# gafniguy/4D-Facial-Avatars

Hardware: AMD Instinct MI355X
Metric: rays/sec at 512x512, 64 coarse + 128 fine samples (higher is better)
Workload: dtype f32; 1 GPU; configs[1]: paper-model eval forward, 512x512 frame, 64+128 samples, chunksize 65536, perturb on, expression+latent conditioned, background prior; frames sharded over GPUs

## Files before the change

### 4d-facial-avatars_amd/build.py

```python
from __future__ import annotations

import os
import shutil
import subprocess
import sys

HERE = os.path.dirname(os.path.abspath(__file__))
SRC = os.path.join(HERE, "csrc")
OUT_DIR = os.path.join(HERE, "lib")
OUT = os.path.join(OUT_DIR, "libnerface_hip.so")
SOURCES = ["nf_lib.hip", "nf_rays.hip", "nf_choice.hip", "nf_render.hip", "nf_render_bwd_full.hip", "nf_mlp.hip", "nf_mlp_bwd.hip", "nf_mlp_bf16.hip", "nf_mlp_f16.hip", "nf_mlp_f16x2.hip", "nf_mlp_f16_train.hip", "nf_mlp_f16_bwd.hip", "nf_mlp_f16_dw.hip", "nf_mlp_bf16_train.hip", "nf_mlp_bf16_bwd.hip", "nf_mlp_bf16_dw.hip", "nf_tiny.hip", "nf_flex.hip", "nf_mlp_lcode.hip", "nf_mlp_lcode_bwd.hip", "nf_mlp_lcode_bf16.hip", "nf_mlp_lcode_f16.hip", "nf_mlp_lcode_f16x2.hip", "nf_mlp_lcode_f16_train.hip", "nf_mlp_lcode_f16_bwd.hip", "nf_mlp_lcode_bf16_train.hip", "nf_mlp_lcode_bf16_bwd.hip", "nf_mlp_bshape.hip", "nf_mlp_cbshape.hip", "nf_mlp_smaller.hip", "nf_mlp_smaller_bwd.hip", "nf_pipeline.hip", "nf_mlp_encoded.hip", "nf_optim.hip", "nf_metrics.hip",
           "nf_mlp_sigma.hip", "nf_mlp_sigma_bf16.hip", "nf_mlp_sigma_f16.hip", "nf_mlp_sigma_f16x2.hip", "nf_mlp_lcode_sigma.hip",
           "nf_mlp_lcode_sigma_bf16.hip", "nf_mlp_lcode_sigma_f16.hip", "nf_mlp_lcode_sigma_f16x2.hip", "nf_mlp_smaller_sigma.hip",
           "nf_mlp_live.hip",
           "nf_mlp_live_stats.hip",
           "nf_mlp_gated.hip", "nf_mlp_gated_stats.hip",
           "nf_isosurface.hip",
           "nf_sparse_grid.hip",
           "nf_mesh_components.hip"]
FLAGS = ["--offload-arch=gfx950", "-O3", "-std=c++17", "-ffp-contract=off", "-fPIC", "-fvisibility=default",
         "-Wno-unused-result"]


UNIT_FLAGS = {u: ["-fno-slp-vectorize"] for u in ("nf_mlp_f16.hip", "nf_mlp_f16x2.hip", "nf_mlp_f16_train.hip", "nf_mlp_lcode_f16.hip",
                                                  "nf_mlp_lcode_f16x2.hip", "nf_mlp_lcode_f16_train.hip", "nf_mlp_sigma_f16.hip",
                                                  "nf_mlp_sigma_f16x2.hip", "nf_mlp_lcode_sigma_f16.hip", "nf_mlp_lcode_sigma_f16x2.hip")}
UNIT_FLAGS.update({u: ["-mllvm", "-amdgpu-atomic-optimizer-strategy=None"] for u in ("nf_mlp_live.hip", "nf_mlp_live_stats.hip",
                                                                                            "nf_mlp_gated.hip", "nf_mlp_gated_stats.hip")})


def _hipcc() -> str:
    for cand in (os.environ.get("HIPCC"), shutil.which("hipcc"), "/opt/rocm/bin/hipcc"):
        if cand and os.path.exists(cand):
            return cand
    raise RuntimeError("hipcc not found (need ROCm's hipcc to build libnerface_hip.so)")


def _stale() -> bool:
    if not os.path.exists(OUT):
        return True
    t = os.path.getmtime(OUT)
    deps = [os.path.join(SRC, f) for f in os.listdir(SRC)] + [os.path.join(HERE, "..", "include", "nerface_hip.h"), __file__]
    return any(os.path.getmtime(d) > t for d in deps)


def _includes(src: str, seen=None) -> set:
    import re
    seen = set() if seen is None else seen
    if src in seen or not os.path.exists(src):
        return seen
    seen.add(src)
    for m in re.finditer(r'^\s*#\s*include\s+"([^"]+)"', open(src).read(), re.M):
        _includes(os.path.normpath(os.path.join(os.path.dirname(src), m.group(1))), seen)
    return seen


def build(force: bool = False, verbose: bool = True) -> str:
    if not force and not _stale():
        return OUT
    os.makedirs(OUT_DIR, exist_ok=True)
    obj_dir = os.path.join(OUT_DIR, "obj")
    os.makedirs(obj_dir, exist_ok=True)
    objs = []
    cc = _hipcc()
    procs = []
    for s in SOURCES:
        src = os.path.join(SRC, s)
        if not os.path.exists(src):
            continue
        obj = os.path.join(obj_dir, s.replace(".hip", ".o"))
        objs.append(obj)
        newest = max(os.path.getmtime(d) for d in _includes(src) | {os.path.abspath(__file__)})
        if not force and os.path.exists(obj) and os.path.getmtime(obj) > newest:
            continue
        procs.append((s, subprocess.Popen([cc, *FLAGS, *UNIT_FLAGS.get(s, []), "-Rpass-analysis=kernel-resource-usage", "-c", src, "-o", obj],
                                          stdout=subprocess.PIPE, stderr=subprocess.STDOUT)))
    for s, p in procs:
        try:
            out, _ = p.communicate(timeout=900)
        except subprocess.TimeoutExpired:
            p.kill()
            raise RuntimeError(f"hipcc timed out on {s}")
        if p.returncode != 0:
            raise RuntimeError(f"hipcc failed on {s}:\n{out.decode()}")
        text = out.decode()
        usage = [ln for ln in text.splitlines() if "-Rpass-analysis=kernel-resource-usage" in ln]
        with open(os.path.join(obj_dir, s.replace(".hip", ".usage.txt")), "w") as f:
            f.write("\n".join(usage) + "\n")
        rest = "\n".join(ln for ln in text.splitlines() if "kernel-resource-usage" not in ln and not ln.lstrip().startswith(("|", "^", "In file included from"))
                         and not ln.strip()[:1].isdigit())
        if verbose and rest.strip():
            print(rest)
    cmd = [cc, "--offload-arch=gfx950", "-shared", "-fPIC", *objs, "-o", OUT]
    r = subprocess.run(cmd, stdout=subprocess.PIPE, stderr=subprocess.STDOUT)
    if r.returncode != 0:
        raise RuntimeError("link failed:\n" + r.stdout.decode())
    if verbose:
        print("built", OUT)
    return OUT


def build_tools(verbose: bool = True):
    micro = os.path.normpath(os.path.join(HERE, "..", "tools", "micro"))
    built = []
    for name in ("store_bw",):
        src, exe = os.path.join(micro, name + ".hip"), os.path.join(micro, name)
        if os.path.exists(exe) and os.path.getmtime(exe) > os.path.getmtime(src):
            continue
        r = subprocess.run([_hipcc(), "--offload-arch=gfx950", "-O2", "-Wno-unused-result", "-o", exe, src], stdout=subprocess.PIPE, stderr=subprocess.STDOUT)
        if r.returncode != 0:
            raise RuntimeError(f"hipcc failed on {src}:\n" + r.stdout.decode())
        built.append(exe)
        if verbose:
            print("built", exe)
    return built


if __name__ == "__main__":
    build(force="--force" in sys.argv)
    build_tools()
```

### 4d-facial-avatars_amd/csrc/nf_mlp_live_kernel.h

```cpp
#pragma once
#include <mutex>
#include "nf_mlp_paper_net.h"

#define NF_LIVE_ROWS 64
#ifndef NF_LIVE_PF
#define NF_LIVE_PF 8
#endif
#define NF_LIVE_DIR_B (NF_LIVE_ROWS * 1024)
#define NF_LIVE_META_B (NF_LIVE_DIR_B + NF_LIVE_ROWS * 64)
#define NF_LIVE_WAVE_B (NF_LIVE_META_B + NF_LIVE_ROWS * 16)
#define NF_LIVE_OOB NF_LIVE_WAVE_B
#define NF_LIVE_SC1 16

static_assert(NF_LIVE_ROWS == 64 && NF_MLP_NT == 2, "row numbers wrap with & 63; a pass's liveness is one 32-bit mask");
static_assert(NF_LIVE_PF >= 0 && NF_LIVE_PF <= 16, "prefetched rows live in registers beside fc_alpha's weights");

__device__ __forceinline__ __amdgpu_buffer_rsrc_t nf_live_ring(char* ring_v) {
    const uint64_t a = (uint64_t)ring_v;
    const uint64_t s = (uint64_t)(uint32_t)__builtin_amdgcn_readfirstlane((int)(uint32_t)a) |
                       ((uint64_t)(uint32_t)__builtin_amdgcn_readfirstlane((int)(a >> 32)) << 32);
    return __builtin_amdgcn_make_buffer_rsrc(reinterpret_cast<char*>(s), (short)0, NF_LIVE_WAVE_B, 0x00020000);
}
__device__ __forceinline__ void nf_live_store(__amdgpu_buffer_rsrc_t ring, int off_b, f32x4 v) {
    __builtin_amdgcn_raw_buffer_store_b128(__builtin_bit_cast(nf_u32x4, v), ring, off_b, 0, 0);
}
__device__ __forceinline__ f32x4 nf_live_load(__amdgpu_buffer_rsrc_t ring, int off_b) {
    return __builtin_bit_cast(f32x4, __builtin_amdgcn_raw_buffer_load_b128(ring, off_b, 0, NF_LIVE_SC1));
}
__device__ __forceinline__ int nf_live_pop(unsigned& m) {
    const int r = __builtin_ctz(m);
    m &= m - 1u;
    return r;
}
__device__ __forceinline__ int nf_live_slab(int prow, int lane) { return nf_act_idx4(prow, lane); }

struct NfLivePre {
    NfStream<NF_MLP_NT>& st;
    f32x4 (&wd)[16];
    f32x4 (&pf)[NF_LIVE_PF > 0 ? NF_LIVE_PF : 1];
    char* ring_v;
    int head_v, tail_v;
    __device__ __forceinline__ void wait() const {
        __builtin_amdgcn_fence(__ATOMIC_RELEASE, "workgroup");
        __builtin_amdgcn_s_waitcnt(0x0F70);
        __builtin_amdgcn_fence(__ATOMIC_ACQUIRE, "workgroup");
    }
    __device__ __forceinline__ void loads(const NfW& Wi, const NfW& Ci, int lane) {
        using Net = NfPaperNet;
        const __amdgpu_buffer_rsrc_t ring = nf_live_ring(ring_v);
        const int tail = __builtin_amdgcn_readfirstlane(tail_v), cnt = __builtin_amdgcn_readfirstlane(head_v) - tail;
#pragma unroll
        for (int i = 0; i < NF_LIVE_PF; ++i)
            pf[i] = nf_live_load(ring, i < cnt ? ((tail + i) & (NF_LIVE_ROWS - 1)) * 1024 + lane * 16 : NF_LIVE_OOB);
        nf_load_bias<8>(st.bias, Ci, Net::B_D0, lane);
        nf_load_w16<8>(st.wa, Wi, Net::OFF_D0 / 4, lane);
        nf_load_w16<8>(wd, Wi, Net::OFF_D0 / 4 + 16 * 9 * 64, lane);
        __builtin_amdgcn_sched_barrier(0);
    }
};

struct NfGatePre {
    NfStream<NF_MLP_NT>& st;
    f32x4 (&pf)[NF_LIVE_PF > 0 ? NF_LIVE_PF : 1];
    char* ring_v;
    int head_v, tail_v;
    const float* bound_v;
    __device__ __forceinline__ NfW image() const {
        const uint64_t a = (uint64_t)bound_v;
        const uint64_t s = (uint64_t)(uint32_t)__builtin_amdgcn_readfirstlane((int)(uint32_t)a) |
                           ((uint64_t)(uint32_t)__builtin_amdgcn_readfirstlane((int)(a >> 32)) << 32);
        return nf_w_image(reinterpret_cast<const float*>(s), NF_BOUND_FLOATS);
    }
    __device__ __forceinline__ void wait() const {
        __builtin_amdgcn_fence(__ATOMIC_RELEASE, "workgroup");
        __builtin_amdgcn_s_waitcnt(0x0F70);
        __builtin_amdgcn_fence(__ATOMIC_ACQUIRE, "workgroup");
    }
    __device__ __forceinline__ void loads(const NfW& Wi, const NfW& Ci, int lane) {
        using Net = NfPaperNet;
        const __amdgpu_buffer_rsrc_t ring = nf_live_ring(ring_v);
        const int tail = __builtin_amdgcn_readfirstlane(tail_v), cnt = __builtin_amdgcn_readfirstlane(head_v) - tail;
#pragma unroll
        for (int i = 0; i < NF_LIVE_PF; ++i)
            pf[i] = nf_live_load(ring, i < cnt ? ((tail + i) & (NF_LIVE_ROWS - 1)) * 1024 + lane * 16 : NF_LIVE_OOB);
        nf_load_bias<16>(st.bias, Ci, Net::B_FEAT, lane);
        nf_load_w16<16>(st.wa, Wi, Net::OFF_FEAT / 4, lane);
        __builtin_amdgcn_sched_barrier(0);
    }
};

#define NF_LIVE_STAT_UNITS 0
#define NF_LIVE_STAT_RUNS 1
#define NF_LIVE_STAT_FLUSH 2
#define NF_LIVE_STAT_CLOCK 3
#define NF_GATE_STAT_PROVEN 4
#define NF_LIVE_PH_TRUNK 0
#define NF_LIVE_PH_TILE 1
#define NF_LIVE_PH_APPEND 2
#define NF_LIVE_PH_ENTRY 3
#define NF_LIVE_PH_RUN 4
#define NF_LIVE_PH_DEAD 5
#define NF_LIVE_PHASES 6
#define NF_LIVE_STAT_COLS 4
#define NF_GATE_STAT_COLS 5

template <bool STATS, int COLS = NF_LIVE_STAT_COLS>
__device__ __forceinline__ void nf_live_stat(long long* stats, int col, long long add, bool set = false) {
    if constexpr (STATS) {
        const int cols = COLS + (((uintptr_t)stats & 1) ? NF_LIVE_PHASES : 0);
        stats = reinterpret_cast<long long*>((uintptr_t)stats & ~(uintptr_t)7);
        if ((threadIdx.x & 63) == 0) {
            long long* at = stats + ((size_t)blockIdx.x * NF_MLP_WAVES + (threadIdx.x >> 6)) * cols + col;
            if (set) *at = add;
            else (void)__hip_atomic_fetch_add(at, add, __ATOMIC_RELAXED, __HIP_MEMORY_SCOPE_AGENT);
        }
    }
}

template <bool STATS, int COLS>
__device__ __forceinline__ void nf_live_mark(long long* stats, int end, int start) {
    if constexpr (STATS) {
        if ((uintptr_t)stats & 1) {
            __builtin_amdgcn_sched_barrier(0);
            const long long t = (long long)__builtin_amdgcn_s_memtime();
            if ((threadIdx.x & 63) == 0) {
                long long* row = reinterpret_cast<long long*>((uintptr_t)stats & ~(uintptr_t)7) +
                                 ((size_t)blockIdx.x * NF_MLP_WAVES + (threadIdx.x >> 6)) * (COLS + NF_LIVE_PHASES) + COLS;
                if (end >= 0) (void)__hip_atomic_fetch_add(row + end, t, __ATOMIC_RELAXED, __HIP_MEMORY_SCOPE_AGENT);
                if (start >= 0) (void)__hip_atomic_fetch_add(row + start, -t, __ATOMIC_RELAXED, __HIP_MEMORY_SCOPE_AGENT);
            }
            __builtin_amdgcn_sched_barrier(0);
        }
    }
}
template <class Pre, int COLS>
struct NfMarkedPre : Pre {
    long long* stats;
    __device__ __forceinline__ void wait() const {
        nf_live_mark<true, COLS>(stats, NF_LIVE_PH_TRUNK, NF_LIVE_PH_TILE);
        Pre::wait();
    }
};

template <int NT, bool STATS, bool GATE = false>
__global__ void __launch_bounds__(64 * NF_MLP_WAVES, 1)
k_paper_mlp_fwd_live(const float* __restrict__ packed, const float* __restrict__ cond_, const float* __restrict__ ro,
                     const float* __restrict__ rd, const float* __restrict__ rd_view, const float* __restrict__ z,
                     int64_t n_points, int S, float* __restrict__ raw, float* __restrict__ scratch, unsigned* __restrict__ counter,
                     long long* __restrict__ stats, const float* __restrict__ bound) {
    using Net = NfPaperNet;
    constexpr int COLS = GATE ? NF_GATE_STAT_COLS : NF_LIVE_STAT_COLS;
    __shared__ __attribute__((aligned(16))) f32x4 lds[NF_MLP_WAVES * 16 * NT * 64];
    const int lane = threadIdx.x & 63, wave = threadIdx.x >> 6;
    f32x4* act4 = lds + wave * (16 * NT * 64);
    typedef __attribute__((address_space(1))) f32x4 nf_gf32x4;
    nf_gf32x4* raw_v = (nf_gf32x4*)raw;
    asm volatile("" : "+v"(raw_v));
    char* ring_v = reinterpret_cast<char*>(scratch) + ((size_t)blockIdx.x * NF_MLP_WAVES + wave) * NF_LIVE_WAVE_B;
    asm volatile("" : "+v"(ring_v));
    const float* z_v = z;
    const float* rdv_v = rd_view;
    asm volatile("" : "+v"(z_v), "+v"(rdv_v));
    const float* bound_v = bound;
    if constexpr (GATE) asm volatile("" : "+v"(bound_v));
    int head_v = 0, tail_v = 0;
    asm volatile("" : "+v"(head_v), "+v"(tail_v));
    typedef __attribute__((address_space(1))) unsigned nf_gu32;
    nf_gu32* ctr_v = (nf_gu32*)counter;
    asm volatile("" : "+v"(ctr_v));
    unsigned unit_v = 0;
    if (lane == 0) unit_v = __hip_atomic_fetch_add(ctr_v, 1u, __ATOMIC_RELAXED, __HIP_MEMORY_SCOPE_AGENT);
    asm volatile("" : "+v"(unit_v));
#pragma unroll 1
    for (;;) {
        const int64_t p0 = (int64_t)(uint32_t)__builtin_amdgcn_readfirstlane((int)unit_v) * (16 * NT);
        int64_t p0_v = p0;
        asm volatile("" : "+v"(p0_v));
        int more_v = p0 < n_points;
        asm volatile("" : "+v"(more_v));
        const bool more = __builtin_amdgcn_readfirstlane(more_v) != 0;
        unsigned next_v = 0;
        if (more && lane == 0) next_v = __hip_atomic_fetch_add(ctr_v, 1u, __ATOMIC_RELAXED, __HIP_MEMORY_SCOPE_AGENT);
        if (more) nf_live_stat<STATS, COLS>(stats, NF_LIVE_STAT_UNITS, 1);
        int opaque0 = 0;
        asm volatile("" : "+s"(opaque0));
        const NfW Wi = nf_w_image(packed + opaque0, Net::PACKED), Ci = nf_w_image(cond_ + opaque0, Net::COND_FLOATS);
        NfStream<NT> st;
        f32x4 wd[16], pf[NF_LIVE_PF > 0 ? NF_LIVE_PF : 1];
        f32x4 dirf[NT][1];
        float sigma_own[NT];
        float tag_own[NT] = {};
        bool proven[NT] = {};
        int live_v = 0, run_v = 0;
        if (more) {
            nf_live_mark<STATS, COLS>(stats, -1, NF_LIVE_PH_TRUNK);
            f32x4 pe[NT][4];
            nf_net_inputs<NT>(pe, dirf, p0, n_points, S, lane, ro, rd, rdv_v, z_v);
            f32x4 acc[NT][16];
            if constexpr (GATE) {
                if constexpr (STATS)
                    nf_paper_net_body<Net, NT, 1, true, NfMarkedPre<NfGatePre, COLS>, true>(
                        acc, sigma_own, pe, dirf, Wi, Ci, act4, lane, NfMarkedPre<NfGatePre, COLS>{{st, pf, ring_v, head_v, tail_v, bound_v}, stats});
                else
                    nf_paper_net_body<Net, NT, 1, true, NfGatePre, true>(acc, sigma_own, pe, dirf, Wi, Ci, act4, lane,
                                                                         NfGatePre{st, pf, ring_v, head_v, tail_v, bound_v});
#pragma unroll
                for (int t = 0; t < NT; ++t) {
                    const float s = acc[t][8].x, u = acc[t][8].y;
                    sigma_own[t] = nf_add(s, nf_mul(u, 0x1p-13f));
                    proven[t] = sigma_own[t] < -0x1p-100f && s > -INFINITY && u < INFINITY;
                }
            } else if constexpr (STATS) {
                nf_paper_net_body<Net, NT, 1, true>(acc, sigma_own, pe, dirf, Wi, Ci, act4, lane,
                                                    NfMarkedPre<NfLivePre, COLS>{{st, wd, pf, ring_v, head_v, tail_v}, stats});
            } else {
                nf_paper_net_body<Net, NT, 1, true>(acc, sigma_own, pe, dirf, Wi, Ci, act4, lane, NfLivePre{st, wd, pf, ring_v, head_v, tail_v});
            }
            nf_live_mark<STATS, COLS>(stats, NF_LIVE_PH_TILE, NF_LIVE_PH_APPEND);
            int lane_o = lane;
            asm volatile("" : "+v"(lane_o));
            const int g = lane_o >> 4, c = lane_o & 15;
            unsigned live = 0;
            int S_o = S;
            asm volatile("" : "+v"(S_o));
            const int64_t p0_o = (int64_t)(uint32_t)__builtin_amdgcn_readfirstlane((int)(uint32_t)p0_v) |
                                 ((int64_t)__builtin_amdgcn_readfirstlane((int)(p0_v >> 32)) << 32);
#pragma unroll
            for (int t = 0; t < NT; ++t) {
                const int64_t p = p0_o + 16 * t + c;
                bool is_live;
                if constexpr (GATE) {
                    const bool last = (p + 1) % S_o == 0;
                    is_live = g == 0 && p < n_points && (!proven[t] || last);
                    tag_own[t] = __int_as_float(last ? 1 : 0);
                } else {
                    is_live = g == 0 && p < n_points && (!(sigma_own[t] <= 0.0f) || (p + 1) % S_o == 0);
                }
                live |= ((unsigned)__builtin_amdgcn_ballot_w64(is_live) & 0xffffu) << (16 * t);
            }
            const int head = __builtin_amdgcn_readfirstlane(head_v), cnt = head - __builtin_amdgcn_readfirstlane(tail_v);
            const int n_live = __builtin_popcount(live);
            live_v = (int)live;
            if constexpr (GATE) {
                const int64_t left = n_points - p0_o;
                nf_live_stat<STATS, COLS>(stats, NF_GATE_STAT_PROVEN, (left < 16 * NT ? (int)left : 16 * NT) - n_live);
            }
            if (cnt + n_live >= 16 * NT) {
                run_v = 1;
            } else {
                const __amdgpu_buffer_rsrc_t ring = nf_live_ring(ring_v);
                unsigned mm = live;
#pragma unroll 1
                for (int i = 0; i < n_live; i += 4) {
                    f32x4 v[4];
                    int off[4];
#pragma unroll
                    for (int u = 0; u < 4; ++u) {
                        const bool ok = i + u < n_live;
                        const int r = ok ? nf_live_pop(mm) : 0;
                        off[u] = ok ? ((head + i + u) & (NF_LIVE_ROWS - 1)) * 1024 + lane_o * 16 : NF_LIVE_OOB;
                        v[u] = act4[nf_live_slab(r, lane_o)];
                    }
#pragma unroll
                    for (int u = 0; u < 4; ++u) nf_live_store(ring, off[u], v[u]);
                }
#pragma unroll
                for (int t = 0; t < NT; ++t) {
                    const int bit = 16 * t + c;
                    if ((live >> bit) & 1u) {
                        const int row = (head + __builtin_popcount(live & ((1u << bit) - 1u))) & (NF_LIVE_ROWS - 1);
                        nf_live_store(ring, NF_LIVE_DIR_B + row * 64 + g * 16, dirf[t][0]);
                        if (g == 0) {
                            const int64_t p = p0_o + bit;
                            nf_live_store(ring, NF_LIVE_META_B + row * 16,
                                          (f32x4){__int_as_float((int)(uint32_t)p), __int_as_float((int)(p >> 32)), GATE ? tag_own[t] : sigma_own[t], 0.0f});
                        }
                    }
                }
                head_v = head + n_live;
                asm volatile("" : "+v"(head_v));
            }
            nf_live_mark<STATS, COLS>(stats, NF_LIVE_PH_APPEND, -1);
        } else {
            if constexpr (GATE) {
                NfGatePre pre{st, pf, ring_v, head_v, tail_v, bound_v};
                pre.wait();
                pre.loads(Wi, Ci, lane);
            } else {
                NfLivePre pre{st, wd, pf, ring_v, head_v, tail_v};
                pre.wait();
                pre.loads(Wi, Ci, lane);
            }
#pragma unroll
            for (int t = 0; t < NT; ++t) {
                dirf[t][0] = (f32x4){0.0f, 0.0f, 0.0f, 0.0f};
                sigma_own[t] = 0.0f;
            }
            run_v = __builtin_amdgcn_readfirstlane(head_v) != __builtin_amdgcn_readfirstlane(tail_v) ? 2 : 0;
        }
        asm volatile("" : "+v"(live_v), "+v"(run_v));
        const int run = __builtin_amdgcn_readfirstlane(run_v);
        if (run != 0) {
            nf_live_stat<STATS, COLS>(stats, NF_LIVE_STAT_RUNS, 1);
            if (run == 2) nf_live_stat<STATS, COLS>(stats, NF_LIVE_STAT_FLUSH, __builtin_amdgcn_readfirstlane(head_v) - __builtin_amdgcn_readfirstlane(tail_v));
            nf_live_mark<STATS, COLS>(stats, -1, NF_LIVE_PH_ENTRY);
            int lane_o = lane;
            asm volatile("" : "+v"(lane_o));
            const int g = lane_o >> 4, c = lane_o & 15;
            const __amdgpu_buffer_rsrc_t ring = nf_live_ring(ring_v);
            const int tail = __builtin_amdgcn_readfirstlane(tail_v), cnt = __builtin_amdgcn_readfirstlane(head_v) - tail;
            const unsigned own = run == 1 ? (unsigned)__builtin_amdgcn_readfirstlane(live_v) : 0u;
            const unsigned fill = run == 1 ? ~own : (1u << cnt) - 1u;
            const int n_fill = __builtin_popcount(fill);
            f32x4 meta[NT];
            bool valid[NT];
#pragma unroll
            for (int t = 0; t < NT; ++t) {
                const int bit = 16 * t + c;
                const bool f = (fill >> bit) & 1u;
                const int row = (tail + __builtin_popcount(fill & ((1u << bit) - 1u))) & (NF_LIVE_ROWS - 1);
                const f32x4 fd = nf_live_load(ring, f ? NF_LIVE_DIR_B + row * 64 + g * 16 : NF_LIVE_OOB);
                const f32x4 fm = nf_live_load(ring, f ? NF_LIVE_META_B + row * 16 : NF_LIVE_OOB);
                const int64_t p = (p0_v) + bit;
                dirf[t][0] = f ? fd : dirf[t][0];
                meta[t] = f ? fm : (f32x4){__int_as_float((int)(uint32_t)p), __int_as_float((int)(p >> 32)), GATE ? tag_own[t] : sigma_own[t], 0.0f};
                valid[t] = f || ((own >> bit) & 1u);
            }
            unsigned hh = fill;
#pragma unroll
            for (int i = 0; i < NF_LIVE_PF; ++i) {
                if (i < n_fill) {
                    const int h = nf_live_pop(hh);
                    act4[nf_live_slab(h, lane_o)] = pf[i];
                }
            }
#pragma unroll 1
            for (int i = NF_LIVE_PF; i < n_fill; i += 4) {
                f32x4 v[4];
                int h[4];
#pragma unroll
                for (int u = 0; u < 4; ++u) {
                    const bool ok = i + u < n_fill;
                    h[u] = ok ? nf_live_pop(hh) : -1;
                    v[u] = nf_live_load(ring, ok ? ((tail + i + u) & (NF_LIVE_ROWS - 1)) * 1024 + lane_o * 16 : NF_LIVE_OOB);
                }
#pragma unroll
                for (int u = 0; u < 4; ++u)
                    if (h[u] >= 0) act4[nf_live_slab(h[u], lane_o)] = v[u];
            }
            constexpr int NDIR = 1;
            constexpr unsigned D0 = Net::OFF_D0 / 4;
            nf_read_b<NT>(st.b0, act4, lane, 0);
            nf_live_mark<STATS, COLS>(stats, NF_LIVE_PH_ENTRY, NF_LIVE_PH_RUN);
            f32x4 acc[NT][16], bj[NT];
            float sigma_raw[NT];
            if constexpr (GATE) {
                nf_seg_lds<NT, 16, true, true>(acc, st, Wi, Net::OFF_FEAT / 4, 16, act4, lane);
                nf_pending_b<NT, true>(bj, st);
                nf_tail<NT, 16, 16, 9, 1>(acc, st.wb, bj, st, Wi, D0, Ci, Net::B_D0, act4, lane);
                NF_NET_COLOUR();
            } else {
                NF_NET_COLOUR_D0(8, 9, wd);
                NF_NET_COLOUR_REST();
            }
            int lane_s = lane;
            asm volatile("" : "+v"(lane_s));
            if ((lane_s >> 4) == 0) {
#pragma unroll
                for (int t = 0; t < NT; ++t) {
                    if (valid[t]) {
                        const int64_t p = (int64_t)(uint32_t)__float_as_int(meta[t].x) | ((int64_t)__float_as_int(meta[t].y) << 32);
                        if constexpr (GATE) {
                            const bool keep = !(sigma_raw[t] <= 0.0f) || __float_as_int(meta[t].z) != 0;
                            if (p >= 0 && p < n_points)
                                raw_v[p] = (f32x4){keep ? acc[t][0].x : 0.0f, keep ? acc[t][0].y : 0.0f, keep ? acc[t][0].z : 0.0f, sigma_raw[t]};
                        } else {
                            if (p >= 0 && p < n_points) raw_v[p] = (f32x4){acc[t][0].x, acc[t][0].y, acc[t][0].z, meta[t].z};
                        }
                    }
                }
            }
            tail_v = tail + n_fill;
            asm volatile("" : "+v"(tail_v));
            nf_live_mark<STATS, COLS>(stats, NF_LIVE_PH_RUN, -1);
        }
        asm volatile("" : "+v"(more_v));
        if (__builtin_amdgcn_readfirstlane(more_v) == 0) break;
        {
            nf_live_mark<STATS, COLS>(stats, -1, NF_LIVE_PH_DEAD);
            int lane_s = lane;
            asm volatile("" : "+v"(lane_s));
            const int g = lane_s >> 4, c = lane_s & 15;
            asm volatile("" : "+v"(live_v));
#pragma unroll
            for (int t = 0; t < NT; ++t) {
                const int64_t p = p0_v + 16 * t + c;
                if (g == 0 && p < n_points && !(((unsigned)live_v >> (16 * t + c)) & 1u)) raw_v[p] = (f32x4){0.0f, 0.0f, 0.0f, sigma_own[t]};
            }
            nf_live_mark<STATS, COLS>(stats, NF_LIVE_PH_DEAD, -1);
        }
        asm volatile("" : "+v"(next_v));
        unit_v = next_v;
    }
    nf_live_stat<STATS, COLS>(stats, NF_LIVE_STAT_CLOCK, (long long)wall_clock64(), true);
}

static inline int64_t nf_live_grid_cap(int max_workgroups) {
    const int64_t cu = nf_cu_count();
    return max_workgroups > 0 && max_workgroups < cu ? max_workgroups : cu;
}

#define NF_LIVE_SLOTS 256
#define NF_LIVE_SLOT_B 128

inline unsigned* nf_live_counter(hipStream_t stream) {
    struct Pool {
        char* base;
        const void* owner[NF_LIVE_SLOTS];
        int used;
    };
    static std::mutex mu;
    static Pool pools[64];
    static thread_local char this_thread;
    int dev = 0;
    if (hipGetDevice(&dev) != hipSuccess || dev < 0 || dev >= 64) return nullptr;
    const void* key = stream == hipStreamPerThread ? (const void*)&this_thread : (const void*)stream;
    std::lock_guard<std::mutex> lock(mu);
    Pool& p = pools[dev];
    if (!p.base) {
        void* mem = nullptr;
        if (hipMalloc(&mem, (size_t)NF_LIVE_SLOTS * NF_LIVE_SLOT_B) != hipSuccess) {
            (void)hipGetLastError();
            return nullptr;
        }
        p.base = (char*)mem;
        p.used = 0;
    }
    int i = 0;
    while (i < p.used && p.owner[i] != key) ++i;
    if (i == p.used) {
        if (p.used == NF_LIVE_SLOTS) {
            if (hipDeviceSynchronize() != hipSuccess) return nullptr;
            p.used = i = 0;
        }
        p.owner[p.used++] = key;
    }
    return reinterpret_cast<unsigned*>(p.base + (size_t)i * NF_LIVE_SLOT_B);
}

template <bool STATS, bool GATE = false>
static inline int nf_live_launch(const float* packed, const float* cond, const float* ro, const float* rd, const float* rd_view, const float* z,
                                 int64_t n_rays, int n_samples, float* raw, float* scratch, size_t scratch_floats, int max_workgroups,
                                 long long* stats, nf_stream_t stream, const float* bound = nullptr, bool clocks = false) {
    static_assert(NF_MLP_WAVES * 16 * NF_MLP_NT == 128, "nf_mlp_fwd_launch sizes the grid for 128 points per workgroup");
    if (max_workgroups < 0 || !scratch || ((uintptr_t)scratch & 15) ||
        scratch_floats < (size_t)nf_live_grid_cap(max_workgroups) * NF_MLP_WAVES * (NF_LIVE_WAVE_B / 4) ||
        (GATE && (!bound || ((uintptr_t)bound & 15))))
        return NF_EINVAL;
    const float* rdv = rd_view ? rd_view : rd;
    if (STATS && clocks) stats = reinterpret_cast<long long*>((uintptr_t)stats | 1);
    int rc = 0;
    const int launched = nf_mlp_fwd_launch(NF_FWD_INFER, packed, cond, ro, rd, z, raw, nullptr, n_rays, n_samples, [&](int64_t n_points, unsigned grid) {
        if ((n_points + 31) / 32 > ((int64_t)1 << 31)) {
            rc = NF_EINVAL;
            return;
        }
        unsigned* counter = nf_live_counter(nf_s(stream));
        if (!counter) {
            rc = (int)hipErrorOutOfMemory;
            return;
        }
        const hipError_t e = hipMemsetAsync(counter, 0, sizeof(unsigned), nf_s(stream));
        if (e != hipSuccess) {
            rc = (int)e;
            return;
        }
        const int64_t cap = nf_live_grid_cap(max_workgroups);
        hipLaunchKernelGGL((k_paper_mlp_fwd_live<NF_MLP_NT, STATS, GATE>), dim3((unsigned)(grid < cap ? grid : cap)), dim3(64 * NF_MLP_WAVES), 0,
                           nf_s(stream), packed, cond, ro, rd, rdv, z, n_points, n_samples, raw, scratch, counter, stats, bound);
    });
    return rc ? rc : launched;
}
```

### 4d-facial-avatars_amd/nerf/_hip.py

```python
from __future__ import annotations

import ctypes as C
import os
import threading

import torch

_LIB_PATH = os.environ.get("NERFACE_HIP_LIB") or os.path.join(os.path.dirname(os.path.dirname(os.path.abspath(__file__))), "lib",
                                                             "libnerface_hip.so")
_lib = None
_lock = threading.Lock()

NF_PAPER_NUM_PARAMS = 26

_P, _I, _L, _F, _Z = C.c_void_p, C.c_int, C.c_int64, C.c_float, C.c_size_t
_PROTOTYPES = {
    "nf_abi_version": (C.c_int, []),
    "nf_error_string": (C.c_char_p, [_I]),
    "nf_build_info": (C.c_char_p, []),
    "nf_ray_bundle": (C.c_int, [_I, _I, _F, _F, _F, _F, _P, _I, _P, _P, _P]),
    "nf_weighted_choice_workspace_bytes": (_Z, []),
    "nf_weighted_choice": (C.c_int, [_P, _P, _L, _I, _P, _P, _Z, _P]),
    "nf_ray_batch": (C.c_int, [_I, _I, _F, _F, _F, _F, _P, _I, _P, _I, _L, _P, _I, _P, _P, _P, _P, _P, _P, _P]),
    "nf_sample_coarse": (C.c_int, [_L, _I, _F, _F, _P, _P, _P, _P]),
# ... 16 lines not shown
    "nf_paper_mlp_fwd_f16x2": (C.c_int, [_P, _P, _P, _P, _P, _P, _L, _I, _P, _P]),
    "nf_paper_mlp_fwd_train_f16": (C.c_int, [_P, _P, _P, _P, _P, _P, _L, _I, _P, _P, _P]),
    "nf_paper_packed_bwd_f16_bytes": (_Z, []),
    "nf_paper_pack_bwd_f16": (C.c_int, [_P, _P, _P]),
    "nf_paper_mlp_bwd_f16": (C.c_int, [_P, _P, _P, _P, _P, _L, _I, _P, _Z, _P, _P]),
    "nf_paper_mlp_fwd_train_bf16": (C.c_int, [_P, _P, _P, _P, _P, _P, _L, _I, _P, _P, _P]),
    "nf_paper_saved_floats": (_Z, [_L]),
    "nf_paper_mlp_fwd_train": (C.c_int, [_P, _P, _P, _P, _P, _P, _L, _I, _P, _P, _P]),
    "nf_paper_packed_bwd_floats": (_Z, []),
    "nf_paper_pack_bwd": (C.c_int, [_P, _P, _P]),
    "nf_paper_packed_bwd_bf16_bytes": (_Z, []),
    "nf_paper_pack_bwd_bf16": (C.c_int, [_P, _P, _P]),
    "nf_paper_mlp_bwd_bf16": (C.c_int, [_P, _P, _P, _P, _P, _L, _I, _P, _Z, _P, _I, _P, _P]),
    "nf_split_saved_to_f32": (C.c_int, [_I, _P, _L, _I, _P, _P]),
    "nf_paper_grad_floats": (_Z, []),
    "nf_paper_bwd_workspace_floats": (_Z, [_L]),
    "nf_paper_mlp_bwd": (C.c_int, [_P, _P, _P, _P, _P, _L, _I, _P, _Z, _P, _P]),
    "nf_paper_mlp_bwd_stage_ms": (C.c_int, [_P, _P, _I, _P, _P, _P, _L, _I, _P, _Z, _P, _P, _P]),
    "nf_lcode_packed_floats": (_Z, []),
    "nf_lcode_cond_floats": (_Z, []),
    "nf_lcode_pack": (C.c_int, [_P, _P, _P]),
    "nf_lcode_condition": (C.c_int, [_P, _P, _P, _F, _F, _P, _P]),
    "nf_lcode_mlp_fwd": (C.c_int, [_P, _P, _P, _P, _P, _P, _L, _I, _P, _P]),
    "nf_lcode_packed_bf16_bytes": (_Z, []),
    "nf_lcode_pack_bf16": (C.c_int, [_P, _P, _P]),
    "nf_lcode_mlp_fwd_bf16": (C.c_int, [_P, _P, _P, _P, _P, _P, _L, _I, _P, _P]),
    "nf_lcode_packed_f16_bytes": (_Z, []),
    "nf_lcode_f16_flag_offset": (_Z, []),
    "nf_lcode_pack_f16": (C.c_int, [_P, _P, _P]),
    "nf_lcode_mlp_fwd_f16": (C.c_int, [_P, _P, _P, _P, _P, _P, _L, _I, _P, _P]),
    "nf_lcode_mlp_fwd_f16x2": (C.c_int, [_P, _P, _P, _P, _P, _P, _L, _I, _P, _P]),
    "nf_lcode_mlp_fwd_train_f16": (C.c_int, [_P, _P, _P, _P, _P, _P, _L, _I, _P, _P, _P]),
    "nf_lcode_packed_bwd_f16_bytes": (_Z, []),
    "nf_lcode_pack_bwd_f16": (C.c_int, [_P, _P, _P]),
    "nf_lcode_mlp_bwd_f16": (C.c_int, [_P, _P, _P, _P, _P, _L, _I, _P, _Z, _P, _P]),
    "nf_lcode_mlp_fwd_train_bf16": (C.c_int, [_P, _P, _P, _P, _P, _P, _L, _I, _P, _P, _P]),
    "nf_lcode_packed_bwd_bf16_bytes": (_Z, []),
    "nf_lcode_pack_bwd_bf16": (C.c_int, [_P, _P, _P]),
    "nf_lcode_mlp_bwd_bf16": (C.c_int, [_P, _P, _P, _P, _P, _L, _I, _P, _Z, _P, _P]),
    "nf_selftest_dw_tables_f32": (C.c_int, []),
    "nf_selftest_dw_tables_lcode_f32": (C.c_int, []),
    "nf_selftest_dw_tables_bf16": (C.c_int, []),
    "nf_paper_stream_table_bf16": (C.c_long, [_P, _Z]),
    "nf_paper_stream_table_bwd_bf16": (C.c_long, [_P, _Z]),
    "nf_lcode_stream_table_bf16": (C.c_long, [_P, _Z]),
    "nf_lcode_stream_table_bwd_bf16": (C.c_long, [_P, _Z]),
    "nf_lcode_forward_encoded": (C.c_int, [_P, _P, _P, _P, _L, _P, _P, _P]),
    "nf_lcode_saved_floats": (_Z, [_L]),
    "nf_lcode_mlp_fwd_train": (C.c_int, [_P, _P, _P, _P, _P, _P, _L, _I, _P, _P, _P]),
    "nf_lcode_packed_bwd_floats": (_Z, []),
    "nf_lcode_pack_bwd": (C.c_int, [_P, _P, _P]),
    "nf_lcode_grad_floats": (_Z, []),
    "nf_lcode_bwd_workspace_floats": (_Z, [_L]),
    "nf_lcode_mlp_bwd": (C.c_int, [_P, _P, _P, _P, _P, _L, _I, _P, _Z, _P, _P]),
    "nf_smaller_packed_floats": (_Z, []),
    "nf_smaller_cond_floats": (_Z, []),
    "nf_smaller_gather_table": (C.c_int, [_P, _Z]),
    "nf_smaller_pack": (C.c_int, [_P, _P, _P]),
    "nf_smaller_condition": (C.c_int, [_P, _P, _P, _F, _F, _P, _P]),
    "nf_smaller_mlp_fwd": (C.c_int, [_P, _P, _P, _P, _P, _P, _L, _I, _P, _P]),
    "nf_smaller_forward_encoded": (C.c_int, [_P, _P, _P, _P, _L, _P, _P, _P]),
    "nf_smaller_saved_floats": (_Z, [_L]),
    "nf_smaller_mlp_fwd_train": (C.c_int, [_P, _P, _P, _P, _P, _P, _L, _I, _P, _P, _P]),
    "nf_smaller_packed_bwd_floats": (_Z, []),
    "nf_smaller_pack_bwd": (C.c_int, [_P, _P, _P]),
    "nf_smaller_grad_floats": (_Z, []),
    "nf_smaller_bwd_workspace_floats": (_Z, [_L]),
    "nf_smaller_mlp_bwd": (C.c_int, [_P, _P, _P, _P, _P, _L, _I, _P, _Z, _P, _P]),
    "nf_smaller_mlp_bwd_stage_ms": (C.c_int, [_P, _P, _P, _P, _P, _L, _I, _P, _Z, _P, _P, _P]),
    "nf_selftest_dw_tables_smaller_f32": (C.c_int, []),
    "nf_eval_postprocess": (C.c_int, [_P, _P, _P, _I, _I, _F, _F, _F, _F, _P, _P, _P]),
    "nf_tiny_packed_floats": (_Z, []),
    "nf_tiny_pack": (C.c_int, [_P, _P, _P]),
    "nf_tiny_mlp_fwd": (C.c_int, [_P, _P, _P, _P, _I, _L, _I, _P, _P]),
    "nf_render_volume_density": (C.c_int, [_P, _P, _L, _I, _P, _P, _P, _P]),
    "nf_tiny_saved_floats": (_Z, [_L]),
    "nf_tiny_mlp_fwd_train": (C.c_int, [_P, _P, _P, _P, _I, _L, _I, _P, _P, _P]),
    "nf_render_volume_density_bwd": (C.c_int, [_P, _P, _P, _L, _I, _P, _P]),
    "nf_render_volume_density_bwd_full": (C.c_int, [_P, _P, _P, _P, _P, _L, _I, _P, _P]),
    "nf_tiny_packed_bwd_floats": (_Z, []),
    "nf_tiny_pack_bwd": (C.c_int, [_P, _P, _P]),
    "nf_tiny_grad_floats": (_Z, []),
    "nf_tiny_bwd_workspace_floats": (_Z, [_L]),
    "nf_tiny_mlp_bwd": (C.c_int, [_P, _P, _P, _L, _I, _P, _Z, _P, _P]),
    "nf_selftest_dw_tables_tiny": (C.c_int, []),
    "nf_flex_packed_floats": (_Z, [_I]),
    "nf_flex_pack": (C.c_int, [_I, _P, _P, _P]),
    "nf_flex_mlp_fwd": (C.c_int, [_I, _P, _P, _P, _P, _I, _L, _I, _P, _P]),
    "nf_flex_saved_floats": (_Z, [_I, _L]),
    "nf_flex_mlp_fwd_train": (C.c_int, [_I, _P, _P, _P, _P, _I, _L, _I, _P, _P, _P]),
    "nf_flex_packed_bwd_floats": (_Z, [_I]),
    "nf_flex_pack_bwd": (C.c_int, [_I, _P, _P, _P]),
    "nf_flex_grad_floats": (_Z, [_I]),
    "nf_flex_bwd_workspace_floats": (_Z, [_I, _L]),
    "nf_flex_mlp_bwd": (C.c_int, [_I, _P, _P, _P, _L, _I, _P, _Z, _P, _P]),
    "nf_selftest_dw_tables_flex": (C.c_int, [_I]),
    "nf_volume_render_fwd": (C.c_int, [_P, _P, _P, _P, _P, _L, _I, _I, _P, _P, _P, _P, _P]),
    "nf_volume_render_bwd": (C.c_int, [_P, _P, _P, _P, _P, _P, _L, _I, _I, _P, _P]),
    "nf_volume_render_bwd_full": (C.c_int, [_P, _P, _P, _P, _P, _P, _P, _P, _P, _P, _L, _I, _I, _P, _P, _P]),
    "nf_sample_pdf": (C.c_int, [_P, _P, _P, _L, _L, _I, _I, _P, _P]),
    "nf_sample_pdf_ex": (C.c_int, [_P, _P, _P, _L, _L, _I, _I, _P, _P, _P, _P]),
    "nf_resample_merge": (C.c_int, [_P, _P, _P, _L, _L, _I, _I, _P, _P, _P]),
    "nf_render_rays_workspace_floats": (_Z, [_L, _I, _I]),
    "nf_render_rays_fwd": (C.c_int, [_P] * 13 + [_L, _P, _P, _L, _I, _I, _F, _F, _I, _P, _Z] + [_P] * 7 + [_P]),
    "nf_render_rays_fwd_f16": (C.c_int, [_P] * 13 + [_L, _P, _P, _L, _I, _I, _F, _F, _I, _P, _Z] + [_P] * 7 + [_P]),
    "nf_render_rays_fwd_f16x2": (C.c_int, [_P] * 13 + [_L, _P, _P, _L, _I, _I, _F, _F, _I, _P, _Z] + [_P] * 7 + [_P]),
    "nf_adam_step": (C.c_int, [_P, _P, _P, _P, _P, _I, _F, _F, _F, _F, _L, _P]),
    "nf_train_loss_fwd": (C.c_int, [_P, _P, _P, _L, _P, _I, _F, _F, _P, _P]),
    "nf_train_loss_bwd": (C.c_int, [_P, _P, _P, _L, _P, _I, _F, _F, _P, _P, _P, _P, _P, _P]),
    "nf_adam_step_dev": (C.c_int, [_P, _P, _P, _P, _P, _I, _F, _F, _F, _P, _P]),
    "nf_train_loss_bg_fwd": (C.c_int, [_P, _P, _P, _L, _P, _I, _F, _F, _P, _P, _F, _P, _P]),
    "nf_train_loss_bg_bwd": (C.c_int, [_P, _P, _P, _L, _P, _I, _F, _F, _P, _P, _F, _P, _P, _P, _P, _P, _P, _P, _P]),
    "nf_sort_rows": (C.c_int, [_P, _L, _I, _P, _P]),
    "nf_image_metrics_workspace_bytes": (_Z, [_L, _I, _I]),
    "nf_image_metrics": (C.c_int, [_P, _P, _L, _I, _I, C.c_double, _P, _Z, _P, _P, _P]),
}
_FAMILY_ENTRY_POINTS = {
    "packed_floats": (_Z, []), "cond_floats": (_Z, []), "pack": (C.c_int, [_P, _P, _P]),
    "condition": (C.c_int, [_P, _P, _P, _F, _F, _P, _P]),
    "mlp_fwd": (C.c_int, [_P, _P, _P, _P, _P, _P, _L, _I, _P, _P]), "mlp_fwd_bf16": (C.c_int, [_P, _P, _P, _P, _P, _P, _L, _I, _P, _P]),
    "mlp_fwd_f16": (C.c_int, [_P, _P, _P, _P, _P, _P, _L, _I, _P, _P]), "mlp_fwd_f16x2": (C.c_int, [_P, _P, _P, _P, _P, _P, _L, _I, _P, _P]),
    "saved_floats": (_Z, [_L]),
    "mlp_fwd_train": (C.c_int, [_P, _P, _P, _P, _P, _P, _L, _I, _P, _P, _P]),
    "mlp_fwd_train_bf16": (C.c_int, [_P, _P, _P, _P, _P, _P, _L, _I, _P, _P, _P]),
    "mlp_fwd_train_f16": (C.c_int, [_P, _P, _P, _P, _P, _P, _L, _I, _P, _P, _P]),
    "packed_bwd_floats": (_Z, []), "pack_bwd": (C.c_int, [_P, _P, _P]),
    "packed_bf16_bytes": (_Z, []), "pack_bf16": (C.c_int, [_P, _P, _P]),
    "packed_bwd_bf16_bytes": (_Z, []), "pack_bwd_bf16": (C.c_int, [_P, _P, _P]),
    "packed_f16_bytes": (_Z, []), "pack_f16": (C.c_int, [_P, _P, _P]),
    "packed_bwd_f16_bytes": (_Z, []), "pack_bwd_f16": (C.c_int, [_P, _P, _P]),
    "f16_flag_offset": (_Z, []),
    "bwd_workspace_floats": (_Z, [_L]), "grad_floats": (_Z, []),
    "mlp_bwd": (C.c_int, [_P, _P, _P, _P, _P, _L, _I, _P, _Z, _P, _P]),
    "mlp_bwd_bf16": (C.c_int, [_P, _P, _P, _P, _P, _L, _I, _P, _Z, _P, _P]),
    "mlp_bwd_f16": (C.c_int, [_P, _P, _P, _P, _P, _L, _I, _P, _Z, _P, _P]),
    "forward_encoded": (C.c_int, [_P, _P, _P, _P, _L, _P, _P, _P]),
}
for _prefix in ("nf_bshape", "nf_cbshape"):
    _PROTOTYPES.update({f"{_prefix}_{_name}": _sig for _name, _sig in _FAMILY_ENTRY_POINTS.items()})
_SIGMA_SIG = (C.c_int, [_P, _P, _P, _P, _P, _P, _L, _I, _P, _P])
SIGMA_ENTRY_POINTS = tuple(f"{_prefix}_mlp_sigma{_suffix}" for _prefix in ("nf_paper", "nf_lcode", "nf_bshape", "nf_cbshape")
                           for _suffix in ("", "_bf16", "_f16", "_f16x2")) + ("nf_smaller_mlp_sigma",)
_PROTOTYPES.update({_name: _SIGMA_SIG for _name in SIGMA_ENTRY_POINTS})
_PROTOTYPES["nf_volume_weights_fwd"] = (C.c_int, [_P, _P, _P, _P, _L, _I, _P, _P, _P, _P])
_PROTOTYPES["nf_paper_mlp_fwd_live_scratch_floats"] = (_Z, [_I])
_PROTOTYPES["nf_paper_mlp_fwd_live"] = (C.c_int, [_P, _P, _P, _P, _P, _P, _L, _I, _P, _P, _Z, _I, _P])
_PROTOTYPES["nf_paper_mlp_fwd_live_stats"] = (C.c_int, [_P, _P, _P, _P, _P, _P, _L, _I, _P, _P, _Z, _I, _P, _Z, _P])
_PROTOTYPES["nf_paper_sigma_bound_floats"] = (_Z, [])
_PROTOTYPES["nf_paper_sigma_bound"] = (C.c_int, [_P, _P, _P])
_PROTOTYPES["nf_paper_mlp_fwd_gated"] = (C.c_int, [_P, _P, _P, _P, _P, _P, _P, _L, _I, _P, _P, _Z, _I, _P])
_PROTOTYPES["nf_paper_mlp_fwd_live_phases"] = _PROTOTYPES["nf_paper_mlp_fwd_live_stats"]
_PROTOTYPES["nf_paper_mlp_fwd_gated_stats"] = (C.c_int, [_P, _P, _P, _P, _P, _P, _P, _L, _I, _P, _P, _Z, _I, _P, _Z, _P])
_PROTOTYPES["nf_paper_mlp_fwd_gated_phases"] = _PROTOTYPES["nf_paper_mlp_fwd_gated_stats"]
_PROTOTYPES["nf_isosurface_workspace_bytes"] = (_Z, [_I, _I, _I])
_PROTOTYPES["nf_isosurface_count"] = (C.c_int, [_P, _I, _I, _I, _F, _P, _Z, _P, _P])
_PROTOTYPES["nf_isosurface_emit"] = (C.c_int, [_P, _I, _I, _I, _F, _P, _P, _P, _Z, _P, _L, _P, _L, _P, _P])
_PROTOTYPES["nf_isosurface_table"] = (C.c_int, [_P])
_PROTOTYPES["nf_sparse_grid_workspace_bytes"] = (_Z, [_I, _I, _I, _I])
_PROTOTYPES["nf_sparse_grid_lattice"] = (C.c_int, [_I, _I, _I, _I, _P, _P, _P, _P, _L, _P])
_PROTOTYPES["nf_sparse_grid_classify"] = (C.c_int, [_P, _I, _I, _I, _I, _F, _F, _I, _P, _Z, _P])
_PROTOTYPES["nf_sparse_grid_mark"] = (C.c_int, [_I, _I, _I, _I, _P, _Z, _P, _P])
_PROTOTYPES["nf_sparse_grid_emit"] = (C.c_int, [_P, _I, _I, _I, _I, _P, _P, _P, _Z, _P, _P, _L, _P])
_PROTOTYPES["nf_sparse_grid_scatter"] = (C.c_int, [_P, _P, _L, _P, _I, _I, _I, _P])
_PROTOTYPES["nf_mesh_components_workspace_bytes"] = (_Z, [_L, _L])
_PROTOTYPES["nf_mesh_components_label"] = (C.c_int, [_P, _L, _L, _P, _Z, _P, _P, _P, _P, _P, _P])
_PROTOTYPES["nf_mesh_components_select"] = (C.c_int, [_P, _P, _P, _L, _L, _I, _L, _P, _Z, _P, _P])
_PROTOTYPES["nf_mesh_components_emit"] = (C.c_int, [_P, _P, _P, _P, _P, _P, _L, _L, _P, _Z, _P, _L, _P, _L, _P, _P])
for _prefix in ("nf_lcode", "nf_bshape", "nf_cbshape"):
    _PROTOTYPES[f"{_prefix}_mlp_bwd_stage_ms"] = (C.c_int, [_P, _P, _I, _P, _P, _P, _L, _I, _P, _Z, _P, _P, _P])
_OPTIONAL = set()
ABI_VERSION = 5


def lib_path() -> str:
    return _LIB_PATH


def lib():
    global _lib
    if _lib is not None:
        return _lib
    with _lock:
        if _lib is not None:
            return _lib
        if not os.path.exists(_LIB_PATH):
            raise RuntimeError(
                f"libnerface_hip.so not found at {_LIB_PATH}: build it with `python 4d-facial-avatars_amd/build.py` "
                "(or __graft_entry__.build()).  This package has no CPU / PyTorch fallback.")
        handle = C.CDLL(_LIB_PATH, mode=C.RTLD_GLOBAL)
        for name, (res, args) in _PROTOTYPES.items():
            try:
                fn = getattr(handle, name)
            except AttributeError:
                if name in _OPTIONAL:
                    continue
                raise RuntimeError(f"libnerface_hip.so does not export {name}; rebuild it")
            fn.restype, fn.argtypes = res, args
        if handle.nf_abi_version() != ABI_VERSION:
            raise RuntimeError(f"libnerface_hip.so at {_LIB_PATH} has ABI revision {handle.nf_abi_version()}, this binding needs {ABI_VERSION}: "
                               "rebuild it (python 4d-facial-avatars_amd/build.py --force)")
        _lib = handle
    return _lib


def check(rc: int, what: str) -> None:
    if rc != 0:
        msg = lib().nf_error_string(rc)
        raise RuntimeError(f"{what} failed: {msg.decode() if msg else rc} (code {rc})")


def stream_ptr(device) -> int:
    return int(torch.cuda.current_stream(device).cuda_stream)


def require_device(*tensors) -> torch.device:
    dev = None
    for t in tensors:
        if t is None:
            continue
        if not t.is_cuda:
            raise RuntimeError("nerf (MI355X build): tensors must live on a ROCm device (`device='cuda'`); "
                               "there is no CPU path in this package")
        if t.dtype != torch.float32:
            raise RuntimeError(f"nerf (MI355X build): expected float32 tensors, got {t.dtype}")
        if not t.is_contiguous():
            raise RuntimeError("nerf (MI355X build): internal error, tensor is not contiguous")
        if dev is None:
            dev = t.device
        elif t.device != dev:
            raise RuntimeError("nerf (MI355X build): tensors are on different devices")
    return dev


def ptr(t) -> int:
    return 0 if t is None else int(t.data_ptr())
```

### 4d-facial-avatars_amd/nerf/models.py

```python
from __future__ import annotations

import torch

from . import ops
from .ops import BSHAPE_KEYS, CBSHAPE_KEYS, LCODE_KEYS, SMALLER_KEYS


class _FusedNeRFModel(torch.nn.Module):

    FAMILY: ops.MLPFamily
    NEEDS_LATENT = True

    def hip_param_list(self):
        sd = dict(self.named_parameters())
        return [sd[k] for k in self.FAMILY.keys]

    def hip_weights(self) -> ops.MLPWeights:
        params = self.hip_param_list()
        hw = self.__dict__.get("_hip_weights")
        if hw is None or any(a is not b for a, b in zip(hw._params, params)):
            hw = self._hip_weights = ops.MLPWeights(self.FAMILY, params)
        return hw

    def hip_forward(self, ro, rd, z, rd_view, expr, latent, near, far, need_grad, live_only=False):
        ops.check_conditioning(expr, latent)
        fam, hw, prec = self.FAMILY, self.hip_weights(), ops.get_mlp_precision()
        fam.require_precision(prec)
        if live_only:
            if need_grad or not ops.live_colour_kernel(fam):
                raise ValueError("live_only is an exact-f32 inference option of the families in ops.LIVE_FAMILIES (ops.live_colour_kernel)")
            packed = hw.get()
            if live_only == "gated":
                return ops.mlp_fwd_gated(fam, packed, hw.get_bound(), ops.mlp_condition(fam, packed, expr, latent, near, far), ro, rd, z, rd_view), None
            return ops.mlp_fwd_live(fam, packed, ops.mlp_condition(fam, packed, expr, latent, near, far), ro, rd, z, rd_view), None
        packed = hw.get()
        cond = ops.mlp_condition(fam, packed, expr, latent, near, far)
        if need_grad:
            ops.require_trainable_precision()
            pb = hw.get_bf16() if prec == "bf16x3" else None
            ph = hw.get_f16() if prec == "f16x3" else None
            if ph is not None:
                ops.f16_guard(self, ro, rd, z, rd_view, expr, latent, near, far, training=True)
            raw, (saved,) = ops.mlp_fwd_train(fam, packed, cond, ro, rd, z, rd_view, packed_b=pb, packed_h=ph)
            return raw, (packed, cond, saved, "f16" if ph is not None else pb is not None)
        if prec in ops.F16_MODES:
            ops.f16_guard(self, ro, rd, z, rd_view, expr, latent, near, far, training=False)
        image = {"f32": hw.get, "bf16x3": hw.get_bf16, "f16x3": hw.get_f16, "f16x2": hw.get_f16}[prec]()
        return ops.mlp_fwd(fam, prec, image, cond, ro, rd, z, rd_view), None

    def hip_sigma(self, ro, rd, z, expr, latent, near, far):
        ops.check_conditioning(expr, latent)
        fam, hw, prec = self.FAMILY, self.hip_weights(), ops.get_mlp_precision()
        fam.require_precision(prec)
        packed = hw.get()
        cond = ops.mlp_condition(fam, packed, expr, latent, near, far)
        if prec in ops.F16_MODES:
            ops.f16_guard(self, ro, rd, z, None, expr, latent, near, far, training=False)
        image = {"f32": hw.get, "bf16x3": hw.get_bf16, "f16x3": hw.get_f16, "f16x2": hw.get_f16}[prec]()
        return ops.mlp_sigma(fam, prec, image, cond, ro, rd, z)

    def hip_backward(self, state, z, d_raw):
        packed, cond, saved, split = state
        return ops.mlp_bwd(self.FAMILY, self.hip_weights(), packed, cond, z, d_raw, saved, split=split)

    def forward(self, x, expr=None, latent_code=None, **kwargs):
        if not self.fused_supported() or expr is None or (latent_code is None and self.NEEDS_LATENT):
            raise NotImplementedError("forward() is built for the NeRFace geometry and needs expr and latent_code")
        if latent_code is None:
            latent_code = torch.zeros(32, dtype=torch.float32, device=x.device)
        if torch.is_grad_enabled() and (x.requires_grad or latent_code.requires_grad or any(p.requires_grad for p in self.parameters())):
            raise NotImplementedError(f"{type(self).__name__}.forward has no autograd on the MI355X build: train through "
                                      "nerf.run_one_iter_of_nerf(...), or call forward under torch.no_grad()")
        return ops.mlp_forward_encoded(self.hip_weights(), x, expr, latent_code)


def density(model, points, expr, latent_code=None):
    if not isinstance(model, _FusedNeRFModel) or not model.fused_supported() or (latent_code is None and model.NEEDS_LATENT):
        raise NotImplementedError("density() is built for the NeRFace geometry and needs expr and latent_code")
    if not (torch.is_tensor(points) and points.is_cuda and torch.is_tensor(expr) and expr.is_cuda):
        raise RuntimeError("nerf (MI355X build): tensors must live on a ROCm device (`device='cuda'`); there is no CPU path in this package")
    if points.dim() != 2 or points.shape[1] != 3:
        raise ValueError("expected points of shape (N, 3)")
    if latent_code is None:
        latent_code = torch.zeros(32, dtype=torch.float32, device=points.device)
    if torch.is_grad_enabled() and (points.requires_grad or latent_code.requires_grad or any(p.requires_grad for p in model.parameters())):
        raise NotImplementedError(f"{type(model).__name__}.forward has no autograd on the MI355X build: train through "
                                  "nerf.run_one_iter_of_nerf(...), or call forward under torch.no_grad()")
    n = points.shape[0]
    if n == 0:
        return torch.empty((0,), dtype=torch.float32, device=points.device)
    ro = ops._c(points.detach().to(torch.float32))
    expr = ops._c(expr.detach().to(torch.float32)).reshape(-1)
    latent = ops._c(latent_code.detach().to(torch.float32)).reshape(-1)
    ops.bump_pack_epoch()
    sigma = model.hip_sigma(ro, torch.zeros_like(ro), torch.zeros((n, 1), dtype=torch.float32, device=ro.device), expr, latent, 0.0, 0.0)
    if ops.get_mlp_precision() in ops.F16_MODES:
        ops.check_f16_range(model)
    return sigma.reshape(n)


class ConditionalBlendshapePaperNeRFModel(_FusedNeRFModel):

    FAMILY = ops.PAPER

    def __init__(self, num_layers=8, hidden_size=256, skip_connect_every=4, num_encoding_fn_xyz=6, num_encoding_fn_dir=4,
                 include_input_xyz=True, include_input_dir=True, use_viewdirs=True, include_expression=True,
                 latent_code_dim=32):
        super().__init__()
        include_input_xyz = 3 if include_input_xyz else 0
        include_input_dir = 3 if include_input_dir else 0
        include_expression = 76 if include_expression else 0
        self.dim_xyz = include_input_xyz + 2 * 3 * num_encoding_fn_xyz
        self.dim_dir = include_input_dir + 2 * 3 * num_encoding_fn_dir
        self.dim_expression = include_expression
        self.dim_latent_code = latent_code_dim
        self.use_viewdirs = use_viewdirs
        d_in = self.dim_xyz + self.dim_expression + self.dim_latent_code
        self.layers_xyz = torch.nn.ModuleList()
        self.layers_xyz.append(torch.nn.Linear(d_in, 256))
        for i in range(1, 6):
            self.layers_xyz.append(torch.nn.Linear(d_in + 256 if i == 3 else 256, 256))
        self.fc_feat = torch.nn.Linear(256, 256)
        self.fc_alpha = torch.nn.Linear(256, 1)
        self.layers_dir = torch.nn.ModuleList()
        self.layers_dir.append(torch.nn.Linear(256 + self.dim_dir, 128))
        for _ in range(3):
            self.layers_dir.append(torch.nn.Linear(128, 128))
        self.fc_rgb = torch.nn.Linear(128, 3)
        self.relu = torch.nn.functional.relu

    def fused_supported(self) -> bool:
        return (self.dim_xyz == 63 and self.dim_dir == 24 and self.dim_expression == 76 and self.dim_latent_code == 32
                and self.use_viewdirs)


class ConditionalBlendshapeLearnableCodeNeRFModel(_FusedNeRFModel):

    FAMILY = ops.LCODE

    def __init__(self, num_layers=4, hidden_size=128, skip_connect_every=4, num_encoding_fn_xyz=6, num_encoding_fn_dir=4,
                 include_input_xyz=True, include_input_dir=True, use_viewdirs=True, include_expression=True, latent_code_dim=32):
        super().__init__()
        include_input_xyz = 3 if include_input_xyz else 0
        include_input_dir = 3 if include_input_dir else 0
        include_expression = 76 if include_expression else 0
        self.dim_xyz = include_input_xyz + 2 * 3 * num_encoding_fn_xyz
        self.dim_dir = include_input_dir + 2 * 3 * num_encoding_fn_dir if use_viewdirs else 0
        self.dim_expression = include_expression
        self.skip_connect_every = skip_connect_every
        self.dim_latent_code = latent_code_dim
        self.layers_expr = None
        d_in = self.dim_xyz + self.dim_expression + self.dim_latent_code
        self.layer1 = torch.nn.Linear(d_in, hidden_size)
        self.layers_xyz = torch.nn.ModuleList()
        for i in range(num_layers - 1):
            skip = i % self.skip_connect_every == 0 and i > 0 and i != num_layers - 1
            self.layers_xyz.append(torch.nn.Linear(self.dim_xyz + hidden_size + self.dim_expression + self.dim_latent_code if skip
                                                   else hidden_size, hidden_size))
        self.use_viewdirs = use_viewdirs
        if self.use_viewdirs:
            self.layers_dir = torch.nn.ModuleList()
            self.layers_dir.append(torch.nn.Linear(self.dim_dir + hidden_size, hidden_size // 2))
            self.fc_alpha = torch.nn.Linear(hidden_size, 1)
            self.fc_rgb = torch.nn.Linear(hidden_size // 2, 3)
            self.fc_feat = torch.nn.Linear(hidden_size, hidden_size)
        else:
            self.fc_out = torch.nn.Linear(hidden_size, 4)
        self.relu = torch.nn.functional.relu
        self.sigmoid = torch.sigmoid

    def fused_supported(self) -> bool:
        return (self.use_viewdirs and self.dim_xyz == 63 and self.dim_dir == 24 and self.dim_expression == 76
                and self.dim_latent_code == 32 and self.layer1.out_features == 256 and len(self.layers_xyz) == 3
                and all(l.in_features == 256 for l in self.layers_xyz))


class _BlendshapeNoCodeNeRFModel(_FusedNeRFModel):

    NEEDS_LATENT = False
    DIM_CONDITION: int

    def _build_trunk(self, num_layers, hidden_size, skip_connect_every, num_encoding_fn_xyz, num_encoding_fn_dir, include_input_xyz,
                     include_input_dir, use_viewdirs):
        self.dim_xyz = (3 if include_input_xyz else 0) + 2 * 3 * num_encoding_fn_xyz
        self.dim_dir = (3 if include_input_dir else 0) + 2 * 3 * num_encoding_fn_dir if use_viewdirs else 0
        self.skip_connect_every = skip_connect_every
        self.layer1 = torch.nn.Linear(self.dim_xyz + self.dim_expression, hidden_size)
# ... 131 lines not shown
```

### 4d-facial-avatars_amd/nerf/ops.py

```python
from __future__ import annotations

import ctypes as C
import os
import weakref
from typing import NamedTuple, Optional, Sequence

import numpy as np
import torch

from . import _hip as H

PAPER_KEYS = (
    [f"layers_xyz.{i}.{p}" for i in range(6) for p in ("weight", "bias")]
    + [f"{n}.{p}" for n in ("fc_feat", "fc_alpha") for p in ("weight", "bias")]
    + [f"layers_dir.{i}.{p}" for i in range(4) for p in ("weight", "bias")]
    + [f"fc_rgb.{p}" for p in ("weight", "bias")]
)
LCODE_KEYS = [f"{n}.{p}" for n in ("layer1", "layers_xyz.0", "layers_xyz.1", "layers_xyz.2", "layers_dir.0", "fc_alpha", "fc_rgb", "fc_feat")
              for p in ("weight", "bias")]
SMALLER_KEYS = [f"{n}.{p}" for n in ([f"layers_xyz.{i}" for i in range(5)] + ["fc_feat", "fc_alpha"] + [f"layers_dir.{i}" for i in range(3)]
                                     + ["fc_rgb"]) for p in ("weight", "bias")]
BSHAPE_KEYS = list(LCODE_KEYS)
CBSHAPE_KEYS = [f"layers_expr.{i}.{p}" for i in range(3) for p in ("weight", "bias")] + LCODE_KEYS

# ... 193 lines not shown
CBSHAPE = MLPFamily("nf_cbshape", tuple(CBSHAPE_KEYS), LCODE.hidden, (), False)

_PACK_EPOCH = [0]


def bump_pack_epoch() -> None:
    _PACK_EPOCH[0] += 1


def pack_epoch() -> int:
    return _PACK_EPOCH[0]


class MLPWeights:

    _KINDS = {
        "f32": ("packed_floats", "pack", torch.float32),
        "f32_t": ("packed_bwd_floats", "pack_bwd", torch.float32),
        "bf16": ("packed_bf16_bytes", "pack_bf16", torch.uint8),
        "bf16_t": ("packed_bwd_bf16_bytes", "pack_bwd_bf16", torch.uint8),
        "f16": ("packed_f16_bytes", "pack_f16", torch.uint8),
        "f16_t": ("packed_bwd_f16_bytes", "pack_bwd_f16", torch.uint8),
    }

    def __init__(self, family: MLPFamily, params: Sequence[torch.Tensor]):
        assert len(params) == len(family.keys)
        self.family = family
        self._params = list(params)
        self._cache = {}
        self._f16_sticky = None

    def invalidate(self) -> None:
        for kind, (_, buf) in list(self._cache.items()):
            self._cache[kind] = (None, buf)

    def _signature(self):
        return (_PACK_EPOCH[0],) + tuple((int(p.data_ptr()), int(p._version)) for p in self._params)

    def _get(self, kind: str) -> torch.Tensor:
        sig = self._signature()
        hit = self._cache.get(kind)
        if hit is None or hit[0] != sig:
            size_fn, pack_fn, dtype = self._KINDS[kind]
            dev = H.require_device(*[p.detach() for p in self._params])
            buf = hit[1] if hit is not None and hit[1].device == dev else torch.empty(self.family.fn(size_fn)(), dtype=dtype, device=dev)
            if kind == "f16" and hit is not None and hit[1] is buf:
                if self._f16_sticky is None or self._f16_sticky.device != dev:
                    self._f16_sticky = torch.zeros((), dtype=torch.int32, device=dev)
                off = self.family.fn("f16_flag_offset")()
                self._f16_sticky.bitwise_or_(buf[off:off + 4].view(torch.int32)[0])
            arr = (C.c_void_p * len(self._params))(*[int(p.data_ptr()) for p in self._params])
            with torch.cuda.device(dev):
                self.family.call(pack_fn, arr, H.ptr(buf), H.stream_ptr(dev))
            self._cache[kind] = (sig, buf)
        return self._cache[kind][1]

    def get(self) -> torch.Tensor:
        return self._get("f32")

    def get_bound(self) -> torch.Tensor:
        packed = self._get("f32")
        sig = self._cache["f32"][0]
        hit = self._cache.get("bound")
        if hit is None or hit[0] != sig or hit[1].device != packed.device:
            self._cache["bound"] = hit = (sig, sigma_bound(self.family, packed))
        return hit[1]

    def get_t(self) -> torch.Tensor:
        return self._get("f32_t")

    def get_bf16(self) -> torch.Tensor:
        return self._get("bf16")

    def get_bf16_t(self) -> torch.Tensor:
        return self._get("bf16_t")

    def get_f16(self) -> torch.Tensor:
        return self._get("f16")

    def get_f16_t(self) -> torch.Tensor:
        return self._get("f16_t")

    def f16_range_flag(self) -> Optional[torch.Tensor]:
        hit = self._cache.get("f16")
        if hit is None:
            return None
        off = self.family.fn("f16_flag_offset")()
        flag = hit[1][off:off + 4].view(torch.int32)[0]
        return flag if self._f16_sticky is None else torch.bitwise_or(flag, self._f16_sticky)


def check_conditioning(expr: torch.Tensor, latent: torch.Tensor) -> None:
    if expr.numel() != 76 or latent.numel() != 32:
        raise ValueError("expected a 76-d expression and a 32-d latent code")


def mlp_condition(fam: MLPFamily, packed, expr, latent, near: float, far: float) -> torch.Tensor:
    expr, latent = _c(expr.detach()), _c(latent.detach())
    dev = H.require_device(packed, expr, latent)
    check_conditioning(expr, latent)
    cond = torch.empty(fam.fn("cond_floats")(), dtype=torch.float32, device=dev)
    with torch.cuda.device(dev):
        fam.call("condition", H.ptr(packed), H.ptr(expr), H.ptr(latent), float(np.float32(near)), float(np.float32(far)), H.ptr(cond),
                 H.stream_ptr(dev))
    return cond


_FWD_ENTRY = {"f32": "mlp_fwd", "bf16x3": "mlp_fwd_bf16", "f16x3": "mlp_fwd_f16", "f16x2": "mlp_fwd_f16x2"}


def mlp_fwd(fam: MLPFamily, precision: str, packed, cond, ro, rd, z, rd_view=None) -> torch.Tensor:
    dev = H.require_device(packed if precision == "f32" else None, cond, ro, rd, z, rd_view)
    n_rays, n_samples = z.shape
    raw = torch.empty((n_rays, n_samples, 4), dtype=torch.float32, device=dev)
    with torch.cuda.device(dev):
        fam.call(_FWD_ENTRY[precision], H.ptr(packed), H.ptr(cond), H.ptr(ro), H.ptr(rd), H.ptr(rd_view), H.ptr(z), n_rays, n_samples,
                 H.ptr(raw), H.stream_ptr(dev))
    return raw


LIVE_FAMILIES = ("nf_paper",)
LIVE_PASSES_DEFAULT = ("coarse", "fine")
_live_passes = set(LIVE_PASSES_DEFAULT)
_live_launches = [0]
_LIVE_SCRATCH = {}
LIVE_RING_ROWS = 64
LIVE_ROW_BYTES = 1024 + 64 + 16
LIVE_PREFETCH_ROWS = 8


def live_rotation_step(workgroups: int) -> int:
    step = (workgroups * 5 // 13) | 1
    return step if step < workgroups else 0


def set_live_colour(on, passes=("coarse", "fine")) -> None:
    global _live_passes, _gated_passes
    _live_passes = set(LIVE_PASSES_DEFAULT) if on is None else (set(passes) if on else set())
    _gated_passes = set(GATED_PASSES_DEFAULT) if on is None else set()


def live_colour_kernel(fam: MLPFamily) -> bool:
    return _mlp_precision == "f32" and fam.prefix in LIVE_FAMILIES


def live_colour_applies(fam: MLPFamily, which: str) -> bool:
    return which in _live_passes and live_colour_kernel(fam)


def live_colour_launches() -> int:
    return _live_launches[0]


def mlp_fwd_live(fam: MLPFamily, packed, cond, ro, rd, z, rd_view=None, max_workgroups: int = 0) -> torch.Tensor:
    if fam.prefix not in LIVE_FAMILIES:
        raise NotImplementedError(f"the {fam.prefix} model family has no live-colour kernel")
    dev = H.require_device(packed, cond, ro, rd, z, rd_view)
    n_rays, n_samples = z.shape
    raw = torch.empty((n_rays, n_samples, 4), dtype=torch.float32, device=dev)
    with torch.cuda.device(dev):
        key = (dev, H.stream_ptr(dev), int(max_workgroups))
        scratch = _LIVE_SCRATCH.get(key)
        if scratch is None:
            scratch = _LIVE_SCRATCH[key] = torch.empty(fam.fn("mlp_fwd_live_scratch_floats")(int(max_workgroups)), dtype=torch.float32, device=dev)
        fam.call("mlp_fwd_live", H.ptr(packed), H.ptr(cond), H.ptr(ro), H.ptr(rd), H.ptr(rd_view), H.ptr(z), n_rays, n_samples, H.ptr(raw),
                 H.ptr(scratch), scratch.numel(), int(max_workgroups), H.stream_ptr(dev))
    _live_launches[0] += 1
    return raw


LIVE_PHASE_COLUMNS = ("clk_trunk", "clk_lone_tile", "clk_append", "clk_run_entry", "clk_run", "clk_dead_stores")
LIVE_STAT_COLUMNS = ("units", "colour_runs", "flush_rows", "exit_clock") + LIVE_PHASE_COLUMNS


def mlp_fwd_live_stats(fam: MLPFamily, packed, cond, ro, rd, z, rd_view=None, max_workgroups: int = 0):
    if fam.prefix not in LIVE_FAMILIES:
        raise NotImplementedError(f"the {fam.prefix} model family has no live-colour kernel")
    dev = H.require_device(packed, cond, ro, rd, z, rd_view)
    n_rays, n_samples = z.shape
    raw = torch.empty((n_rays, n_samples, 4), dtype=torch.float32, device=dev)
    with torch.cuda.device(dev):
        scratch = torch.empty(fam.fn("mlp_fwd_live_scratch_floats")(int(max_workgroups)), dtype=torch.float32, device=dev)
        waves = scratch.numel() * 4 // (LIVE_RING_ROWS * LIVE_ROW_BYTES)
        stats = torch.empty((waves, len(LIVE_STAT_COLUMNS)), dtype=torch.int64, device=dev)
        fam.call("mlp_fwd_live_phases", H.ptr(packed), H.ptr(cond), H.ptr(ro), H.ptr(rd), H.ptr(rd_view), H.ptr(z), n_rays, n_samples,
                 H.ptr(raw), H.ptr(scratch), scratch.numel(), int(max_workgroups), stats.data_ptr(), waves, H.stream_ptr(dev))
    return raw, stats


GATED_PASSES_DEFAULT = ("coarse", "fine")
_gated_passes = (set(GATED_PASSES_DEFAULT) if os.environ.get("NERFACE_SIGMA_GATE") is None
                 else {p for p in os.environ["NERFACE_SIGMA_GATE"].split(",") if p in ("coarse", "fine")})
_gated_launches = [0]
GATED_STAT_COLUMNS = LIVE_STAT_COLUMNS[:4] + ("proven_rows",) + LIVE_PHASE_COLUMNS


def set_sigma_gate(on, passes=("coarse", "fine")) -> None:
    global _gated_passes
    _gated_passes = set(GATED_PASSES_DEFAULT) if on is None else (set(passes) if on else set())


def sigma_gate_applies(fam: MLPFamily, which: str) -> bool:
    return which in _gated_passes and live_colour_kernel(fam)


def live_mode(fam: MLPFamily, which: str):
    if sigma_gate_applies(fam, which):
        return "gated"
    return live_colour_applies(fam, which)


def sigma_gate_launches() -> int:
    return _gated_launches[0]


def sigma_bound(fam: MLPFamily, packed) -> torch.Tensor:
    if fam.prefix not in LIVE_FAMILIES:
        raise NotImplementedError(f"the {fam.prefix} model family has no gated kernel")
    dev = H.require_device(packed)
    bound = torch.empty(fam.fn("sigma_bound_floats")(), dtype=torch.float32, device=dev)
    with torch.cuda.device(dev):
        fam.call("sigma_bound", H.ptr(packed), H.ptr(bound), H.stream_ptr(dev))
    return bound


def _gated_call(entry, fam, packed, bound, cond, ro, rd, z, rd_view, max_workgroups, scratch, raw, *tail):
    n_rays, n_samples = z.shape
    fam.call(entry, H.ptr(packed), H.ptr(bound), H.ptr(cond), H.ptr(ro), H.ptr(rd), H.ptr(rd_view), H.ptr(z), n_rays, n_samples, H.ptr(raw),
             H.ptr(scratch), scratch.numel(), int(max_workgroups), *tail)


def mlp_fwd_gated(fam: MLPFamily, packed, bound, cond, ro, rd, z, rd_view=None, max_workgroups: int = 0) -> torch.Tensor:
    if fam.prefix not in LIVE_FAMILIES:
        raise NotImplementedError(f"the {fam.prefix} model family has no gated kernel")
    dev = H.require_device(packed, bound, cond, ro, rd, z, rd_view)
    n_rays, n_samples = z.shape
    raw = torch.empty((n_rays, n_samples, 4), dtype=torch.float32, device=dev)
    with torch.cuda.device(dev):
        key = (dev, H.stream_ptr(dev), int(max_workgroups))
        scratch = _LIVE_SCRATCH.get(key)
        if scratch is None:
            scratch = _LIVE_SCRATCH[key] = torch.empty(fam.fn("mlp_fwd_live_scratch_floats")(int(max_workgroups)), dtype=torch.float32, device=dev)
        _gated_call("mlp_fwd_gated", fam, packed, bound, cond, ro, rd, z, rd_view, max_workgroups, scratch, raw, H.stream_ptr(dev))
    _gated_launches[0] += 1
    return raw


def mlp_fwd_gated_stats(fam: MLPFamily, packed, bound, cond, ro, rd, z, rd_view=None, max_workgroups: int = 0):
    if fam.prefix not in LIVE_FAMILIES:
        raise NotImplementedError(f"the {fam.prefix} model family has no gated kernel")
    dev = H.require_device(packed, bound, cond, ro, rd, z, rd_view)
    n_rays, n_samples = z.shape
    raw = torch.empty((n_rays, n_samples, 4), dtype=torch.float32, device=dev)
    with torch.cuda.device(dev):
        scratch = torch.empty(fam.fn("mlp_fwd_live_scratch_floats")(int(max_workgroups)), dtype=torch.float32, device=dev)
        waves = scratch.numel() * 4 // (LIVE_RING_ROWS * LIVE_ROW_BYTES)
        stats = torch.empty((waves, len(GATED_STAT_COLUMNS)), dtype=torch.int64, device=dev)
        _gated_call("mlp_fwd_gated_phases", fam, packed, bound, cond, ro, rd, z, rd_view, max_workgroups, scratch, raw, stats.data_ptr(), waves,
                    H.stream_ptr(dev))
    return raw, stats


_SIGMA_ENTRY = {"f32": "mlp_sigma", "bf16x3": "mlp_sigma_bf16", "f16x3": "mlp_sigma_f16", "f16x2": "mlp_sigma_f16x2"}


def mlp_sigma(fam: MLPFamily, precision: str, image, cond, ro, rd, z) -> torch.Tensor:
    dev = H.require_device(image if precision == "f32" else None, cond, ro, rd, z)
    n_rays, n_samples = z.shape
    sigma = torch.empty((n_rays, n_samples), dtype=torch.float32, device=dev)
    with torch.cuda.device(dev):
        fam.call(_SIGMA_ENTRY[precision], H.ptr(image), H.ptr(cond), H.ptr(ro), H.ptr(rd), 0, H.ptr(z), n_rays, n_samples, H.ptr(sigma),
                 H.stream_ptr(dev))
    return sigma


def mlp_fwd_train(fam: MLPFamily, packed, cond, ro, rd, z, rd_view=None, packed_b=None, packed_h=None):
    dev = H.require_device(packed, cond, ro, rd, z, rd_view)
    n_rays, n_samples = z.shape
    raw = torch.empty((n_rays, n_samples, 4), dtype=torch.float32, device=dev)
    saved = torch.empty(fam.fn("saved_floats")(n_rays * n_samples), dtype=torch.float32, device=dev)
    entry, image = (("mlp_fwd_train_f16", packed_h) if packed_h is not None else
                    ("mlp_fwd_train_bf16", packed_b) if packed_b is not None else ("mlp_fwd_train", packed))
    with torch.cuda.device(dev):
        fam.call(entry, H.ptr(image), H.ptr(cond), H.ptr(ro), H.ptr(rd), H.ptr(rd_view), H.ptr(z), n_rays, n_samples, H.ptr(raw),
                 H.ptr(saved), H.stream_ptr(dev))
    return raw, (saved,)


def mlp_bwd(fam: MLPFamily, weights: MLPWeights, packed, cond, z, d_raw, saved_t, split=False, exact_dw=False):
    if exact_dw and not fam.exact_dw:
        raise ValueError(f"exact_dw: the split-bf16 backward of {fam.prefix} has no exact-f32 weight-gradient form")
    d_raw = _c(d_raw)
    dev = H.require_device(packed, cond, saved_t, d_raw)
    n_rays, n_samples = z.shape
    with torch.cuda.device(dev):
        ws_floats = fam.fn("bwd_workspace_floats")(n_rays * n_samples)
    ws = torch.empty(ws_floats, dtype=torch.float32, device=dev)
    flat = torch.empty(fam.fn("grad_floats")(), dtype=torch.float32, device=dev)
    args = (H.ptr(cond), H.ptr(saved_t), H.ptr(d_raw), n_rays, n_samples, H.ptr(ws), ws_floats, H.ptr(flat))
    with torch.cuda.device(dev):
        if split == "f16":
            fam.call("mlp_bwd_f16", H.ptr(packed), H.ptr(weights.get_f16_t()), *args, H.stream_ptr(dev))
        elif split:
            packed_bt, exact = weights.get_bf16_t(), ()
            if fam.exact_dw:
                saved_f32 = split_saved_to_f32(saved_t, n_rays * n_samples, False) if exact_dw else None
                exact = (int(bool(exact_dw)), H.ptr(saved_f32))
            fam.call("mlp_bwd_bf16", H.ptr(packed), H.ptr(packed_bt), *args, *exact, H.stream_ptr(dev))
        else:
            fam.call("mlp_bwd", H.ptr(packed), H.ptr(weights.get_t()), *args, H.stream_ptr(dev))
    grads, off = [], 0
    for i, p in enumerate(weights._params):
        n = p.numel()
        grads.append(None if i in fam.none_grads else flat[off:off + n].view(p.shape))
        off += n
    return grads, flat[off:off + 32]


def mlp_forward_encoded(weights: MLPWeights, x, expr, latent) -> torch.Tensor:
    x = _c(x.detach())
    if x.dim() != 2 or x.shape[1] != 87:
        raise ValueError("expected pre-encoded inputs of shape (N, 87)")
    expr, latent = _c(expr.detach()).reshape(-1), _c(latent.detach()).reshape(-1)
    check_conditioning(expr, latent)
    packed = weights.get()
    dev = H.require_device(packed, x, expr, latent)
    fam = weights.family
    cond = torch.empty(fam.fn("cond_floats")(), dtype=torch.float32, device=dev)
    out = torch.empty((x.shape[0], 4), dtype=torch.float32, device=dev)
    with torch.cuda.device(dev):
        fam.call("forward_encoded", H.ptr(packed), H.ptr(x), H.ptr(expr), H.ptr(latent), x.shape[0], H.ptr(cond), H.ptr(out),
                 H.stream_ptr(dev))
    return out


def paper_condition(packed: torch.Tensor, expr: torch.Tensor, latent: torch.Tensor, near: float, far: float) -> torch.Tensor:
    return mlp_condition(PAPER, packed, expr, latent, near, far)


def paper_mlp_fwd(packed, cond, ro, rd, z, rd_view=None) -> torch.Tensor:
    return mlp_fwd(PAPER, "f32", packed, cond, ro, rd, z, rd_view)


def paper_mlp_fwd_bf16(packed_b, cond, ro, rd, z, rd_view=None) -> torch.Tensor:
    return mlp_fwd(PAPER, "bf16x3", packed_b, cond, ro, rd, z, rd_view)


def paper_mlp_fwd_f16(packed_h, cond, ro, rd, z, rd_view=None) -> torch.Tensor:
    return mlp_fwd(PAPER, "f16x3", packed_h, cond, ro, rd, z, rd_view)


def paper_mlp_fwd_f16x2(packed_h, cond, ro, rd, z, rd_view=None) -> torch.Tensor:
    return mlp_fwd(PAPER, "f16x2", packed_h, cond, ro, rd, z, rd_view)


def paper_mlp_fwd_train(packed, cond, ro, rd, z, rd_view=None, packed_b=None, packed_h=None):
    return mlp_fwd_train(PAPER, packed, cond, ro, rd, z, rd_view, packed_b=packed_b, packed_h=packed_h)


def paper_mlp_bwd(model, packed, cond, z, d_raw, saved, split=False, exact_dw=False):
    (saved_t,) = saved
    return mlp_bwd(PAPER, model.hip_weights(), packed, cond, z, d_raw, saved_t, split=split, exact_dw=exact_dw)


def split_saved_to_f32(saved_t: torch.Tensor, n_points: int, f16: bool, family: str = "paper") -> torch.Tensor:
    fam = LCODE if family == "lcode" else PAPER
    dev = H.require_device(saved_t)
    out = torch.empty(fam.fn("saved_floats")(n_points), dtype=torch.float32, device=dev)
    with torch.cuda.device(dev):
        H.check(H.lib().nf_split_saved_to_f32(int(fam is LCODE), H.ptr(saved_t), n_points, int(bool(f16)), H.ptr(out), H.stream_ptr(dev)),
                "nf_split_saved_to_f32")
    return out


def require_trainable_precision() -> None:
    if _mlp_precision in INFERENCE_ONLY_PRECISIONS:
        raise RuntimeError(f'nerf.set_mlp_precision("{_mlp_precision}") is an inference arithmetic: train with "f32", "f16x3" or "bf16x3"')


_f16_train_probe_every = [128]


def set_f16_train_probe_every(n: int) -> None:
    _f16_train_probe_every[0] = max(1, int(n))


def f16_train_probe_every() -> int:
    return _f16_train_probe_every[0]


F16_ACT_LIMIT = 65504.0 / 16.0
F16_PREFLIGHT_MARGIN = 4.0


def f16_preflight(model, ro, rd, z, rd_view, expr, latent, near, far, max_rays: int = 256, max_samples: int = 8) -> float:
    n_rays, n_s = z.shape
    rs = max(1, n_rays // max_rays)
    ss = max(1, n_s // max_samples)
    ro_s, rd_s = ro[::rs].contiguous(), rd[::rs].contiguous()
    z_s = z[::rs, ::ss].contiguous()
    rv_s = None if rd_view is None else rd_view[::rs].contiguous()
    hw = model.hip_weights()
    packed = hw.get()
    cond = mlp_condition(hw.family, packed, expr, latent, near, far)
    _, (saved,) = mlp_fwd_train(hw.family, packed, cond, ro_s, rd_s, z_s, rv_s)
    lo, hi = hw.family.hidden
    n = z_s.numel()
    return float(saved[lo * n:hi * n].abs().max().item())


def f16_guard(model, ro, rd, z, rd_view, expr, latent, near, far, training: bool) -> None:
    state = model.__dict__
    if training and torch.cuda.is_current_stream_capturing():
# ... 629 lines not shown
```

### 4d-facial-avatars_amd/nerf/train_utils.py

```python
from __future__ import annotations

from typing import Optional

import torch

from . import ops
from .nerf_helpers import PositionalEncoder, get_minibatches
from .volume_rendering_utils import volume_render_radiance_field


def run_network(network_fn, pts, ray_batch, chunksize, embed_fn, embeddirs_fn, expressions=None, latent_code=None):
    pts_flat = pts.reshape((-1, pts.shape[-1]))
    embedded = embed_fn(pts_flat)
    if embeddirs_fn is not None:
        viewdirs = ray_batch[..., None, -3:]
        input_dirs_flat = viewdirs.expand(pts.shape).reshape((-1, 3))
        embedded = torch.cat((embedded, embeddirs_fn(input_dirs_flat.contiguous())), dim=-1)
    batches = get_minibatches(embedded, chunksize=chunksize)
    if expressions is None:
        preds = [network_fn(batch) for batch in batches]
    elif latent_code is not None:
        preds = [network_fn(batch, expressions, latent_code) for batch in batches]
    else:
        preds = [network_fn(batch, expressions) for batch in batches]
    radiance_field = torch.cat(preds, dim=0)
    return radiance_field.reshape(list(pts.shape[:-1]) + [radiance_field.shape[-1]])


def _integrator_backward(raw, z, rd, noise, bg, d_rgb, d_disp, d_acc, d_w_last, white, need_d_bg):
    if d_rgb is None and d_disp is None and d_acc is None and d_w_last is None:
        return None, None
    if d_disp is None and d_acc is None and d_w_last is None and not need_d_bg:
        return ops.volume_render_bwd(raw, z, rd, noise, bg, d_rgb, white), None
    return ops.volume_render_bwd_full(raw, z, rd, noise, bg, ops._c(d_rgb), ops._c(d_disp), ops._c(d_acc), None, ops._c(d_w_last),
                                      white, need_d_bg)


class _RenderChunk(torch.autograd.Function):

    @staticmethod
    def forward(ctx, cfg, ro, rd, rd_view, bg, expr, latent, t_rand, noise_c, u, noise_f, n_params_c, *params):
        model_c, model_f = cfg["model_coarse"], cfg["model_fine"]
        near, far, nc, nf = cfg["near"], cfg["far"], cfg["num_coarse"], cfg["num_fine"]
        white = cfg["white_background"]
        need_grad = cfg["need_grad"]
        ctx.set_materialize_grads(False)
        dev = ro.device
        n_rays = ro.shape[0]

        lat_d = latent.detach().reshape(-1).contiguous()
        live_c = not need_grad and noise_c is None and ops.live_mode(model_c.FAMILY, "coarse")
        live_f = not need_grad and noise_f is None and model_f is not None and ops.live_mode(model_f.FAMILY, "fine")
        z_c = ops.sample_coarse(n_rays, nc, near, far, dev, t_rand, lindisp=cfg["lindisp"])
        if cfg.get("coarse_density_only"):
            raw_c = state_c = rgb_c = None
            disp_c, acc_c, w_c = ops.volume_weights_fwd(model_c.hip_sigma(ro, rd, z_c, expr, lat_d, near, far), z_c, rd, noise_c)
        else:
            raw_c, state_c = model_c.hip_forward(ro, rd, z_c, rd_view, expr, lat_d, near, far, need_grad, live_only=live_c)
            rgb_c, disp_c, acc_c, w_c = ops.volume_render_fwd(raw_c, z_c, rd, noise_c, bg, white)
        outs = [rgb_c, disp_c, acc_c]
        ctx.has_fine = nf > 0 and model_f is not None
        if ctx.has_fine:
            z_f = ops.resample_merge(z_c, w_c, nf, u)
            raw_f, state_f = model_f.hip_forward(ro, rd, z_f, rd_view, expr, lat_d, near, far, need_grad, live_only=live_f)
            rgb_f, disp_f, acc_f, w_f = ops.volume_render_fwd(raw_f, z_f, rd, noise_f, bg, white)
            w_last = w_f[:, -1].contiguous()
            outs += [rgb_f, disp_f, acc_f, w_last]
        else:
            w_last = w_c[:, -1].contiguous()
            outs += [w_last]
        if need_grad:
            ctx.cfg = cfg
            ctx.n_params_c = n_params_c
            ctx.save_for_backward(rd, bg, noise_c, noise_f, z_c, raw_c, latent)
            ctx.state_c = state_c
            if ctx.has_fine:
                ctx.fine = (z_f, raw_f, state_f)
        return tuple(outs)

    @staticmethod
    def backward(ctx, *grads):
        cfg = ctx.cfg
        rd, bg, noise_c, noise_f, z_c, raw_c, latent = ctx.saved_tensors
        model_c, model_f = cfg["model_coarse"], cfg["model_fine"]
        white = cfg["white_background"]
        need_d_bg = bg is not None and ctx.needs_input_grad[4]
        g_latent = g_bg = None
        grads_c = [None] * ctx.n_params_c
        grads_f = []
        d_raw_c, g_bg = _integrator_backward(raw_c, z_c, rd, noise_c, bg, grads[0], grads[1], grads[2],
                                             None if ctx.has_fine else grads[3], white, need_d_bg)
        if d_raw_c is not None:
            grads_c, g_latent = model_c.hip_backward(ctx.state_c, z_c, d_raw_c)
        ctx.state_c = None
        if ctx.has_fine:
            z_f, raw_f, state_f = ctx.fine
            grads_f = [None] * len(model_f.hip_param_list())
            d_raw_f, g_bg_f = _integrator_backward(raw_f, z_f, rd, noise_f, bg, grads[3], grads[4], grads[5], grads[6], white, need_d_bg)
            if d_raw_f is not None:
                grads_f, gl = model_f.hip_backward(state_f, z_f, d_raw_f)
                g_latent = gl if g_latent is None else g_latent + gl
            if g_bg_f is not None:
                g_bg = g_bg_f if g_bg is None else g_bg + g_bg_f
            ctx.fine = None
        g_latent = g_latent.reshape(latent.shape) if (ctx.needs_input_grad[6] and g_latent is not None) else None
        return (None, None, None, None, g_bg, None, g_latent, None, None, None, None, None, *grads_c, *grads_f)


def _check_encoders(encode_position_fn, encode_direction_fn):
    ok = (isinstance(encode_position_fn, PositionalEncoder) and encode_position_fn.num_encoding_functions == 10
          and encode_position_fn.include_input and encode_position_fn.log_sampling
          and isinstance(encode_direction_fn, PositionalEncoder) and encode_direction_fn.num_encoding_functions == 4
          and not encode_direction_fn.include_input and encode_direction_fn.log_sampling)
    if not ok:
        raise NotImplementedError(
            "the fused MLP kernel is built for the NeRFace encoders: get_embedding_function(10, include_input=True) "
            "for positions and get_embedding_function(4, include_input=False) for directions (log sampling)")


def _check_chunk_args(model_coarse, encode_position_fn, encode_direction_fn, expressions, latent_code, rays):
    _check_encoders(encode_position_fn, encode_direction_fn)
    if expressions is None or latent_code is None:
        raise NotImplementedError("the NeRFace path needs `expressions` and `latent_code` (unconditioned NeRF is out of scope)")
    if not getattr(model_coarse, "fused_supported", lambda: False)():
        raise NotImplementedError(f"{type(model_coarse).__name__}: no fused HIP kernel for this model/geometry")
    if not rays.is_cuda:
        raise RuntimeError("nerf (MI355X build): rays must be on a ROCm device; there is no CPU path")


def predict_and_render_radiance(ray_batch, model_coarse, model_fine, options, mode="train", encode_position_fn=None,
                                encode_direction_fn=None, expressions=None, background_prior=None, latent_code=None,
                                ray_dirs_fake=None):
    _check_chunk_args(model_coarse, encode_position_fn, encode_direction_fn, expressions, latent_code, ray_batch)
    n_rays = ray_batch.shape[0]
    rb = ray_batch.to(torch.float32)
    ro = rb[:, 0:3].contiguous()
    rd = rb[:, 3:6].contiguous()
    rd_view = None
    if ray_dirs_fake:
        rd_view = ray_dirs_fake[0][:n_rays, 3:6].to(torch.float32).contiguous()
        ray_batch[..., 3:6] = ray_dirs_fake[0][..., 3:6]
    return _render_rays(ro, rd, rd_view, model_coarse, model_fine, options, mode, expressions, background_prior, latent_code)


def _render_rays(ro, rd, rd_view, model_coarse, model_fine, options, mode, expressions, background_prior, latent_code):
    m = getattr(options.nerf, mode)
    dev = ro.device
    n_rays = ro.shape[0]
    nc, nf = int(m.num_coarse), int(m.num_fine)
    near, far = float(options.dataset.near), float(options.dataset.far)
    has_fine = nf > 0 and model_fine is not None
    noise_std = float(m.radiance_field_noise_std)
    params_c = model_coarse.hip_param_list()
    params_f = model_fine.hip_param_list() if has_fine else []
    need_grad = torch.is_grad_enabled() and (latent_code.requires_grad or any(p.requires_grad for p in params_c + params_f)
                                             or (background_prior is not None and background_prior.requires_grad))
    ops.check_sample_counts(nc, nf if has_fine else 0, need_grad)
    density_only = bool(getattr(m, "coarse_density_only", False))
    if density_only and not has_fine:
        raise ValueError("coarse_density_only needs a fine network (num_fine > 0 and a fine model): the coarse colour would be the image")
    if density_only and need_grad:
        raise ValueError("coarse_density_only is an inference option: call under torch.no_grad() (the density-only kernels have no backward)")
    t_rand = torch.rand((n_rays, nc), dtype=torch.float32, device=dev) if m.perturb else None
    noise_c = (torch.randn((n_rays, nc), dtype=torch.float32, device=dev) * noise_std) if noise_std > 0.0 else None
    u = noise_f = None
    if nf > 0:
        det = (m.perturb == 0.0)
        u = None if det else torch.rand([n_rays, nf], dtype=torch.float32, device=dev)
        if model_fine is not None and noise_std > 0.0:
            noise_f = torch.randn((n_rays, nc + nf), dtype=torch.float32, device=dev) * noise_std
    bg = None
    if background_prior is not None:
        bg = background_prior.to(device=dev, dtype=torch.float32).reshape(-1, 3).contiguous()
    expr = expressions.to(device=dev, dtype=torch.float32).reshape(-1).contiguous()
    cfg = dict(model_coarse=model_coarse, model_fine=model_fine if has_fine else None, near=near, far=far, num_coarse=nc,
               lindisp=bool(m.lindisp),
               num_fine=nf if has_fine else 0, white_background=bool(m.white_background), need_grad=need_grad,
               coarse_density_only=density_only)
    lat = latent_code if latent_code.dtype == torch.float32 else latent_code.to(torch.float32)
    outs = _RenderChunk.apply(cfg, ro, rd, rd_view, bg, expr, lat, t_rand, noise_c, u, noise_f, len(params_c),
                              *params_c, *params_f)
    if has_fine:
        return tuple(outs)
    rgb_c, disp_c, acc_c, w_last = outs
    return rgb_c, disp_c, acc_c, None, None, None, w_last


def run_one_iter_of_nerf(height, width, focal_length, model_coarse, model_fine, ray_origins, ray_directions, options,
                         mode="train", encode_position_fn=None, encode_direction_fn=None, expressions=None,
                         background_prior=None, latent_code=None, ray_directions_ablation=None):
    is_rad = torch.is_tensor(ray_directions_ablation)
    ops.bump_pack_epoch()
    if options.dataset.no_ndc is False:
        raise NotImplementedError("NDC rays are not part of the NeRFace path (all configs use no_ndc: True)")
    restore_shapes = [ray_directions.shape, ray_directions.shape[:-1], ray_directions.shape[:-1]]
    if model_fine:
        restore_shapes += restore_shapes
        restore_shapes += [ray_directions.shape[:-1]]
    ro = ray_origins.reshape((-1, 3))
    rd = ray_directions.reshape((-1, 3))
    chunksize = getattr(options.nerf, mode).chunksize
    bg_chunks = get_minibatches(background_prior, chunksize=chunksize) if background_prior is not None else None
    if is_rad:
        near = options.dataset.near * torch.ones_like(rd[..., :1])
        far = options.dataset.far * torch.ones_like(rd[..., :1])
        rays = torch.cat((ro, rd, near, far), dim=-1)
        batches = get_minibatches(rays, chunksize=chunksize)
        rays_ablation = torch.cat((ro, ray_directions_ablation.reshape((-1, 3)), near, far), dim=-1)
        batches_ablation = get_minibatches(rays_ablation, chunksize=chunksize)
        pred = [
            predict_and_render_radiance(batch, model_coarse, model_fine, options, mode, encode_position_fn=encode_position_fn,
                                        encode_direction_fn=encode_direction_fn, expressions=expressions,
                                        background_prior=bg_chunks[i] if bg_chunks is not None else None,
                                        latent_code=latent_code, ray_dirs_fake=batches_ablation)
            for i, batch in enumerate(batches)
        ]
    else:
# ... 45 lines not shown
```

### include/nerface_hip.h

```cpp
#ifndef NERFACE_HIP_H
#define NERFACE_HIP_H

#include <stddef.h>
#include <stdint.h>

#ifdef __cplusplus
extern "C" {
#endif

typedef void* nf_stream_t;

#define NF_EINVAL (-22)

int         nf_abi_version(void);
const char* nf_error_string(int code);
const char* nf_build_info(void);

int nf_ray_bundle(int height, int width, float fx, float fy, float cx_w, float cy_h,
                  const float* c2w, int c2w_row_stride, float* ro, float* rd, nf_stream_t stream);

int nf_ray_batch(int height, int width, float fx, float fy, float cx_w, float cy_h, const float* c2w, int c2w_row_stride,
                 const int64_t* sel, int sel_is_flat, int64_t n, const float* image, int channels, const float* bg, float* ro,
                 float* rd, float* target, float* bg_out, int* bad_flag, nf_stream_t stream);

// ... 237 lines not shown
                             const float* z, int64_t n_rays, int n_samples, float* raw, float* saved, nf_stream_t stream);
size_t nf_smaller_packed_bwd_floats(void);
int nf_smaller_pack_bwd(const float* const* params, float* packed_t, nf_stream_t stream);
size_t nf_smaller_grad_floats(void);
size_t nf_smaller_bwd_workspace_floats(int64_t n_points);
int nf_smaller_mlp_bwd(const float* packed, const float* packed_t, const float* cond, const float* saved, const float* d_raw,
                       int64_t n_rays, int n_samples, float* workspace, size_t workspace_floats, float* grads,
                       nf_stream_t stream);
int nf_smaller_mlp_bwd_stage_ms(const float* packed, const float* packed_t, const float* cond, const float* saved,
                                const float* d_raw, int64_t n_rays, int n_samples, float* workspace, size_t workspace_floats,
                                float* grads, float* stage_ms, nf_stream_t stream);

size_t nf_tiny_packed_floats(void);
int nf_tiny_pack(const float* const* params, float* packed, nf_stream_t stream);
int nf_tiny_mlp_fwd(const float* packed, const float* ro, const float* rd, const float* depth, int depth_per_ray,
                    int64_t n_rays, int n_samples, float* raw, nf_stream_t stream);
int nf_render_volume_density(const float* raw, const float* depth, int64_t n_rays, int n_samples, float* rgb,
                             float* depth_map, float* acc, nf_stream_t stream);

size_t nf_tiny_saved_floats(int64_t n_points);
int nf_tiny_mlp_fwd_train(const float* packed, const float* ro, const float* rd, const float* depth, int depth_per_ray,
                          int64_t n_rays, int n_samples, float* raw, float* saved, nf_stream_t stream);
int nf_render_volume_density_bwd(const float* raw, const float* depth, const float* d_rgb, int64_t n_rays, int n_samples,
                                 float* d_raw, nf_stream_t stream);
int nf_render_volume_density_bwd_full(const float* raw, const float* depth, const float* d_rgb, const float* d_depth,
                                      const float* d_acc, int64_t n_rays, int n_samples, float* d_raw, nf_stream_t stream);
size_t nf_tiny_packed_bwd_floats(void);
int nf_tiny_pack_bwd(const float* const* params, float* packed_t, nf_stream_t stream);
size_t nf_tiny_grad_floats(void);
size_t nf_tiny_bwd_workspace_floats(int64_t n_points);
int nf_tiny_mlp_bwd(const float* packed_t, const float* saved, const float* d_raw, int64_t n_rays, int n_samples,
                    float* workspace, size_t workspace_floats, float* grads, nf_stream_t stream);

size_t nf_flex_packed_floats(int num_layers);
int nf_flex_pack(int num_layers, const float* const* params, float* packed, nf_stream_t stream);
int nf_flex_mlp_fwd(int num_layers, const float* packed, const float* ro, const float* rd, const float* depth, int depth_per_ray,
                    int64_t n_rays, int n_samples, float* raw, nf_stream_t stream);
size_t nf_flex_saved_floats(int num_layers, int64_t n_points);
int nf_flex_mlp_fwd_train(int num_layers, const float* packed, const float* ro, const float* rd, const float* depth,
                          int depth_per_ray, int64_t n_rays, int n_samples, float* raw, float* saved, nf_stream_t stream);
size_t nf_flex_packed_bwd_floats(int num_layers);
int nf_flex_pack_bwd(int num_layers, const float* const* params, float* packed_t, nf_stream_t stream);
size_t nf_flex_grad_floats(int num_layers);
size_t nf_flex_bwd_workspace_floats(int num_layers, int64_t n_points);
int nf_flex_mlp_bwd(int num_layers, const float* packed_t, const float* saved, const float* d_raw, int64_t n_rays, int n_samples,
                    float* workspace, size_t workspace_floats, float* grads, nf_stream_t stream);

int nf_eval_postprocess(const float* rgb, const float* depthmap, const float* weights, int height, int width, float fx,
                        float fy, float cx_w, float cy_h, uint8_t* rgb_u8, uint8_t* normals_u8, nf_stream_t stream);

size_t nf_image_metrics_workspace_bytes(int64_t n, int height, int width);
int nf_image_metrics(const uint8_t* a, const uint8_t* b, int64_t n, int height, int width, double ssim_range, void* workspace,
                     size_t workspace_bytes, double* out_f64, int64_t* out_i64, nf_stream_t stream);

int nf_sample_pdf(const float* bins, const float* weights, const float* u, int64_t u_row_stride,
                  int64_t n_rays, int n_bins, int n_out, float* samples, nf_stream_t stream);
int nf_sample_pdf_ex(const float* bins, const float* weights, const float* u, int64_t u_row_stride, int64_t n_rays,
                     int n_bins, int n_out, float* samples, int* inds, float* cdf, nf_stream_t stream);

int nf_resample_merge(const float* z_coarse, const float* w_coarse, const float* u, int64_t u_row_stride,
                      int64_t n_rays, int n_coarse, int n_fine, float* z_samples ,
                      float* z_fine , nf_stream_t stream);

size_t nf_render_rays_workspace_floats(int64_t n_rays, int n_coarse, int n_fine);
int nf_render_rays_fwd(const float* packed_coarse, const void* packed_bf16_coarse, const float* packed_fine,
                       const void* packed_bf16_fine, const float* expr76, const float* latent32, const float* ro,
                       const float* rd, const float* rd_view, const float* bg, const float* t_vals, const float* t_rand,
                       const float* u, int64_t u_row_stride, const float* noise_coarse, const float* noise_fine,
                       int64_t n_rays, int n_coarse, int n_fine, float near_z, float far_z, int white_background,
                       float* workspace, size_t workspace_floats, float* rgb_coarse, float* disp_coarse, float* acc_coarse,
                       float* rgb_fine, float* disp_fine, float* acc_fine, float* w_last, nf_stream_t stream);

int nf_render_rays_fwd_f16(const float* packed_coarse, const void* packed_f16_coarse, const float* packed_fine,
                           const void* packed_f16_fine, const float* expr76, const float* latent32, const float* ro,
                           const float* rd, const float* rd_view, const float* bg, const float* t_vals, const float* t_rand,
                           const float* u, int64_t u_row_stride, const float* noise_coarse, const float* noise_fine,
                           int64_t n_rays, int n_coarse, int n_fine, float near_z, float far_z, int white_background,
                           float* workspace, size_t workspace_floats, float* rgb_coarse, float* disp_coarse, float* acc_coarse,
                           float* rgb_fine, float* disp_fine, float* acc_fine, float* w_last, nf_stream_t stream);

int nf_render_rays_fwd_f16x2(const float* packed_coarse, const void* packed_f16_coarse, const float* packed_fine,
                             const void* packed_f16_fine, const float* expr76, const float* latent32, const float* ro,
                             const float* rd, const float* rd_view, const float* bg, const float* t_vals, const float* t_rand,
                             const float* u, int64_t u_row_stride, const float* noise_coarse, const float* noise_fine,
                             int64_t n_rays, int n_coarse, int n_fine, float near_z, float far_z, int white_background,
                             float* workspace, size_t workspace_floats, float* rgb_coarse, float* disp_coarse, float* acc_coarse,
                             float* rgb_fine, float* disp_fine, float* acc_fine, float* w_last, nf_stream_t stream);

int nf_adam_step(float* const* params, const float* const* grads, float* const* exp_avg, float* const* exp_avg_sq,
                 const int64_t* numel, int n_tensors, float lr, float beta1, float beta2, float eps, int64_t step,
                 nf_stream_t stream);

int nf_train_loss_fwd(const float* rgb_coarse, const float* rgb_fine, const float* target, int64_t n_elems, const float* latent,
                      int n_latent, float code_weight, float code_scale, float* out7, nf_stream_t stream);
int nf_train_loss_bwd(const float* rgb_coarse, const float* rgb_fine, const float* target, int64_t n_elems, const float* latent,
                      int n_latent, float code_weight, float code_scale, const float* out7, const float* grad_out,
                      float* d_rgb_coarse, float* d_rgb_fine, float* d_latent, nf_stream_t stream);

int nf_adam_step_dev(float* const* params, const float* const* grads, float* const* exp_avg, float* const* exp_avg_sq,
                     const int64_t* numel, int n_tensors, float beta1, float beta2, float eps, void* state, nf_stream_t stream);
int nf_train_loss_bg_fwd(const float* rgb_coarse, const float* rgb_fine, const float* target, int64_t n_elems, const float* latent,
                         int n_latent, float code_weight, float code_scale, const float* bg, const float* w_last, float bg_weight,
                         float* out8, nf_stream_t stream);
int nf_train_loss_bg_bwd(const float* rgb_coarse, const float* rgb_fine, const float* target, int64_t n_elems, const float* latent,
                         int n_latent, float code_weight, float code_scale, const float* bg, const float* w_last, float bg_weight,
                         const float* out8, const float* grad_out, float* d_rgb_coarse, float* d_rgb_fine, float* d_latent,
                         float* d_bg, float* d_w_last, nf_stream_t stream);

int nf_sort_rows(const float* in, int64_t n_rows, int n_cols, float* out, nf_stream_t stream);

#define NF_DECLARE_MLP_SIGMA(PFX)                                                                                                   \
    int PFX##_mlp_sigma(const float* packed, const float* cond, const float* ro, const float* rd, const float* rd_view,            \
                        const float* z, int64_t n_rays, int n_samples, float* sigma, nf_stream_t stream);
#define NF_DECLARE_MLP_SIGMA_SPLIT(PFX)                                                                                             \
    int PFX##_mlp_sigma_bf16(const void* packed_bf16, const float* cond, const float* ro, const float* rd, const float* rd_view,   \
                             const float* z, int64_t n_rays, int n_samples, float* sigma, nf_stream_t stream);                     \
    int PFX##_mlp_sigma_f16(const void* packed_f16, const float* cond, const float* ro, const float* rd, const float* rd_view,     \
                            const float* z, int64_t n_rays, int n_samples, float* sigma, nf_stream_t stream);                      \
    int PFX##_mlp_sigma_f16x2(const void* packed_f16, const float* cond, const float* ro, const float* rd, const float* rd_view,   \
                              const float* z, int64_t n_rays, int n_samples, float* sigma, nf_stream_t stream);
NF_DECLARE_MLP_SIGMA(nf_paper) NF_DECLARE_MLP_SIGMA_SPLIT(nf_paper)
NF_DECLARE_MLP_SIGMA(nf_lcode) NF_DECLARE_MLP_SIGMA_SPLIT(nf_lcode)
NF_DECLARE_MLP_SIGMA(nf_bshape) NF_DECLARE_MLP_SIGMA_SPLIT(nf_bshape)
NF_DECLARE_MLP_SIGMA(nf_cbshape) NF_DECLARE_MLP_SIGMA_SPLIT(nf_cbshape)
NF_DECLARE_MLP_SIGMA(nf_smaller)
#undef NF_DECLARE_MLP_SIGMA
#undef NF_DECLARE_MLP_SIGMA_SPLIT
int nf_volume_weights_fwd(const float* sigma, const float* z, const float* rd, const float* noise, int64_t n_rays, int n_samples,
                          float* disp, float* acc, float* weights, nf_stream_t stream);

size_t nf_paper_mlp_fwd_live_scratch_floats(int max_workgroups);
int nf_paper_mlp_fwd_live(const float* packed, const float* cond, const float* ro, const float* rd, const float* rd_view,
                          const float* z, int64_t n_rays, int n_samples, float* raw, float* scratch, size_t scratch_floats,
                          int max_workgroups, nf_stream_t stream);
int nf_paper_mlp_fwd_live_phases(const float* packed, const float* cond, const float* ro, const float* rd, const float* rd_view,
                                 const float* z, int64_t n_rays, int n_samples, float* raw, float* scratch, size_t scratch_floats,
                                 int max_workgroups, int64_t* stats, size_t stats_rows, nf_stream_t stream);
int nf_paper_mlp_fwd_live_stats(const float* packed, const float* cond, const float* ro, const float* rd, const float* rd_view,
                                const float* z, int64_t n_rays, int n_samples, float* raw, float* scratch, size_t scratch_floats,
                                int max_workgroups, int64_t* stats, size_t stats_rows, nf_stream_t stream);

int nf_paper_mlp_fwd_gated_phases(const float* packed, const float* bound, const float* cond, const float* ro, const float* rd,
                                  const float* rd_view, const float* z, int64_t n_rays, int n_samples, float* raw, float* scratch,
                                  size_t scratch_floats, int max_workgroups, int64_t* stats, size_t stats_rows, nf_stream_t stream);
size_t nf_paper_sigma_bound_floats(void);
int nf_paper_sigma_bound(const float* packed, float* bound, nf_stream_t stream);
int nf_paper_mlp_fwd_gated(const float* packed, const float* bound, const float* cond, const float* ro, const float* rd,
                           const float* rd_view, const float* z, int64_t n_rays, int n_samples, float* raw, float* scratch,
                           size_t scratch_floats, int max_workgroups, nf_stream_t stream);
int nf_paper_mlp_fwd_gated_stats(const float* packed, const float* bound, const float* cond, const float* ro, const float* rd,
                                 const float* rd_view, const float* z, int64_t n_rays, int n_samples, float* raw, float* scratch,
                                 size_t scratch_floats, int max_workgroups, int64_t* stats, size_t stats_rows, nf_stream_t stream);

size_t nf_isosurface_workspace_bytes(int nx, int ny, int nz);
int nf_isosurface_count(const float* grid, int nx, int ny, int nz, float level, void* workspace, size_t workspace_bytes,
                        int64_t* counts_dev, nf_stream_t stream);
int nf_isosurface_emit(const float* grid, int nx, int ny, int nz, float level, const float* lo, const float* hi, void* workspace,
                       size_t workspace_bytes, float* verts, int64_t n_verts, int* faces, int64_t n_faces, float* normals,
                       nf_stream_t stream);
int nf_isosurface_table(uint32_t* out);

size_t nf_sparse_grid_workspace_bytes(int nx, int ny, int nz, int brick);
int nf_sparse_grid_lattice(int nx, int ny, int nz, int brick, const float* lo, const float* hi, int* index, float* coords,
                           int64_t capacity, nf_stream_t stream);
int nf_sparse_grid_classify(const float* grid, int nx, int ny, int nz, int brick, float level, float margin, int dilate,
                            void* workspace, size_t workspace_bytes, nf_stream_t stream);
int nf_sparse_grid_mark(int nx, int ny, int nz, int brick, void* workspace, size_t workspace_bytes, int64_t* counts_dev,
                        nf_stream_t stream);
int nf_sparse_grid_emit(float* grid, int nx, int ny, int nz, int brick, const float* lo, const float* hi, void* workspace,
                        size_t workspace_bytes, int* index, float* coords, int64_t capacity, nf_stream_t stream);
int nf_sparse_grid_scatter(const float* values, const int* index, int64_t count, float* grid, int nx, int ny, int nz,
                           nf_stream_t stream);

size_t nf_mesh_components_workspace_bytes(int64_t n_vertices, int64_t n_faces);
int nf_mesh_components_label(const int* faces, int64_t n_vertices, int64_t n_faces, void* workspace, size_t workspace_bytes,
                             int* vertex_label, int* face_label, int* face_counts, int* vertex_counts, int64_t* counts_dev,
                             nf_stream_t stream);
int nf_mesh_components_select(const int* vertex_label, const int* face_label, const int* face_counts, int64_t n_vertices,
                              int64_t n_faces, int largest, int64_t min_faces, void* workspace, size_t workspace_bytes,
                              int64_t* counts_dev, nf_stream_t stream);
int nf_mesh_components_emit(const float* vertices, const int* faces, const float* normals, const int* vertex_label,
                            const int* face_label, const int* face_counts, int64_t n_vertices, int64_t n_faces, void* workspace,
                            size_t workspace_bytes, float* out_vertices, int64_t cap_vertices, int* out_faces, int64_t cap_faces,
                            float* out_normals, nf_stream_t stream);

int nf_selftest_dw_tables_f32(void);
int nf_selftest_dw_tables_lcode_f32(void);
int nf_selftest_dw_tables_smaller_f32(void);
int nf_selftest_dw_tables_bf16(void);
int nf_selftest_dw_tables_tiny(void);
int nf_selftest_dw_tables_flex(int num_layers);
long nf_paper_stream_table_bf16(uint32_t* out, size_t n_entries);
long nf_paper_stream_table_bwd_bf16(uint32_t* out, size_t n_entries);
long nf_lcode_stream_table_bf16(uint32_t* out, size_t n_entries);
long nf_lcode_stream_table_bwd_bf16(uint32_t* out, size_t n_entries);

#ifdef __cplusplus
}
#endif
#endif
```

Baseline: 622,500 rays/s.

## Skip MLP evaluation of each ray's last sample when a background prior is used

Adds skip-last kernel variants for the live and gated paper-MLP forward passes. They map point indices so that each ray's final sample (whose colour only feeds the background-composited term) is left out of the network, using a precomputed bound on the network's factors to stay safe. The new path is on by default for both the coarse and fine passes when a background is present. It saves roughly 1/S of the MLP work per ray, but adds extra kernels, a factor-bound launch on every call, and index remapping cost.

```diff
diff --git a/4d-facial-avatars_amd/build.py b/4d-facial-avatars_amd/build.py
--- a/4d-facial-avatars_amd/build.py
+++ b/4d-facial-avatars_amd/build.py
@@ -15,6 +15,7 @@
            "nf_mlp_live.hip",
            "nf_mlp_live_stats.hip",
            "nf_mlp_gated.hip", "nf_mlp_gated_stats.hip",
+           "nf_mlp_skip_last.hip", "nf_mlp_skip_last_stats.hip", "nf_mlp_live_skip.hip", "nf_mlp_live_skip_stats.hip",
            "nf_isosurface.hip",
            "nf_sparse_grid.hip",
            "nf_mesh_components.hip"]
@@ -26,7 +27,9 @@
                                                   "nf_mlp_lcode_f16x2.hip", "nf_mlp_lcode_f16_train.hip", "nf_mlp_sigma_f16.hip",
                                                   "nf_mlp_sigma_f16x2.hip", "nf_mlp_lcode_sigma_f16.hip", "nf_mlp_lcode_sigma_f16x2.hip")}
 UNIT_FLAGS.update({u: ["-mllvm", "-amdgpu-atomic-optimizer-strategy=None"] for u in ("nf_mlp_live.hip", "nf_mlp_live_stats.hip",
-                                                                                            "nf_mlp_gated.hip", "nf_mlp_gated_stats.hip")})
+                                                                                            "nf_mlp_gated.hip", "nf_mlp_gated_stats.hip",
+                                                                                            "nf_mlp_skip_last.hip", "nf_mlp_skip_last_stats.hip",
+                                                                                            "nf_mlp_live_skip.hip", "nf_mlp_live_skip_stats.hip")})
 
 
 def _hipcc() -> str:
diff --git a/4d-facial-avatars_amd/csrc/nf_mlp_live_kernel.h b/4d-facial-avatars_amd/csrc/nf_mlp_live_kernel.h
--- a/4d-facial-avatars_amd/csrc/nf_mlp_live_kernel.h
+++ b/4d-facial-avatars_amd/csrc/nf_mlp_live_kernel.h
@@ -142,268 +142,51 @@
     }
 };
 
-template <int NT, bool STATS, bool GATE = false>
-__global__ void __launch_bounds__(64 * NF_MLP_WAVES, 1)
-k_paper_mlp_fwd_live(const float* __restrict__ packed, const float* __restrict__ cond_, const float* __restrict__ ro,
-                     const float* __restrict__ rd, const float* __restrict__ rd_view, const float* __restrict__ z,
-                     int64_t n_points, int S, float* __restrict__ raw, float* __restrict__ scratch, unsigned* __restrict__ counter,
-                     long long* __restrict__ stats, const float* __restrict__ bound) {
-    using Net = NfPaperNet;
-    constexpr int COLS = GATE ? NF_GATE_STAT_COLS : NF_LIVE_STAT_COLS;
-    __shared__ __attribute__((aligned(16))) f32x4 lds[NF_MLP_WAVES * 16 * NT * 64];
-    const int lane = threadIdx.x & 63, wave = threadIdx.x >> 6;
-    f32x4* act4 = lds + wave * (16 * NT * 64);
-    typedef __attribute__((address_space(1))) f32x4 nf_gf32x4;
-    nf_gf32x4* raw_v = (nf_gf32x4*)raw;
-    asm volatile("" : "+v"(raw_v));
-    char* ring_v = reinterpret_cast<char*>(scratch) + ((size_t)blockIdx.x * NF_MLP_WAVES + wave) * NF_LIVE_WAVE_B;
-    asm volatile("" : "+v"(ring_v));
-    const float* z_v = z;
-    const float* rdv_v = rd_view;
-    asm volatile("" : "+v"(z_v), "+v"(rdv_v));
-    const float* bound_v = bound;
-    if constexpr (GATE) asm volatile("" : "+v"(bound_v));
-    int head_v = 0, tail_v = 0;
-    asm volatile("" : "+v"(head_v), "+v"(tail_v));
-    typedef __attribute__((address_space(1))) unsigned nf_gu32;
-    nf_gu32* ctr_v = (nf_gu32*)counter;
-    asm volatile("" : "+v"(ctr_v));
-    unsigned unit_v = 0;
-    if (lane == 0) unit_v = __hip_atomic_fetch_add(ctr_v, 1u, __ATOMIC_RELAXED, __HIP_MEMORY_SCOPE_AGENT);
-    asm volatile("" : "+v"(unit_v));
-#pragma unroll 1
-    for (;;) {
-        const int64_t p0 = (int64_t)(uint32_t)__builtin_amdgcn_readfirstlane((int)unit_v) * (16 * NT);
-        int64_t p0_v = p0;
-        asm volatile("" : "+v"(p0_v));
-        int more_v = p0 < n_points;
-        asm volatile("" : "+v"(more_v));
-        const bool more = __builtin_amdgcn_readfirstlane(more_v) != 0;
-        unsigned next_v = 0;
-        if (more && lane == 0) next_v = __hip_atomic_fetch_add(ctr_v, 1u, __ATOMIC_RELAXED, __HIP_MEMORY_SCOPE_AGENT);
-        if (more) nf_live_stat<STATS, COLS>(stats, NF_LIVE_STAT_UNITS, 1);
-        int opaque0 = 0;
-        asm volatile("" : "+s"(opaque0));
-        const NfW Wi = nf_w_image(packed + opaque0, Net::PACKED), Ci = nf_w_image(cond_ + opaque0, Net::COND_FLOATS);
-        NfStream<NT> st;
-        f32x4 wd[16], pf[NF_LIVE_PF > 0 ? NF_LIVE_PF : 1];
-        f32x4 dirf[NT][1];
-        float sigma_own[NT];
-        float tag_own[NT] = {};
-        bool proven[NT] = {};
-        int live_v = 0, run_v = 0;
-        if (more) {
-            nf_live_mark<STATS, COLS>(stats, -1, NF_LIVE_PH_TRUNK);
-            f32x4 pe[NT][4];
-            nf_net_inputs<NT>(pe, dirf, p0, n_points, S, lane, ro, rd, rdv_v, z_v);
-            f32x4 acc[NT][16];
-            if constexpr (GATE) {
-                if constexpr (STATS)
-                    nf_paper_net_body<Net, NT, 1, true, NfMarkedPre<NfGatePre, COLS>, true>(
-                        acc, sigma_own, pe, dirf, Wi, Ci, act4, lane, NfMarkedPre<NfGatePre, COLS>{{st, pf, ring_v, head_v, tail_v, bound_v}, stats});
-                else
-                    nf_paper_net_body<Net, NT, 1, true, NfGatePre, true>(acc, sigma_own, pe, dirf, Wi, Ci, act4, lane,
-                                                                         NfGatePre{st, pf, ring_v, head_v, tail_v, bound_v});
+__device__ __forceinline__ uint32_t nf_skip_map(uint32_t p, uint32_t np, uint32_t n_full, int S, bool& last, uint32_t& ray) {
+    const bool full = np == n_full;
+    const uint32_t d = full ? (uint32_t)S : (uint32_t)S - 1u;
+    ray = p / d;
+    last = full && p - ray * d == d - 1u;
+    return full ? p : p + ray;
+}
+
+#define NF_SKIP_LAST_BIT 0x80000000u
+template <int NT>
+__device__ __forceinline__ void nf_net_inputs_skip(f32x4 (&pe)[NT][4], f32x4 (&dirf)[NT][1], uint32_t (&qv)[NT], uint32_t p0, uint32_t np,
+                                                   uint32_t n_full, int S, int lane, const float* __restrict__ ro,
+                                                   const float* __restrict__ rd, const float* __restrict__ rd_view,
+                                                   const float* __restrict__ z) {
+    const int g = lane >> 4, c = lane & 15;
 #pragma unroll
-                for (int t = 0; t < NT; ++t) {
-                    const float s = acc[t][8].x, u = acc[t][8].y;
-                    sigma_own[t] = nf_add(s, nf_mul(u, 0x1p-13f));
-                    proven[t] = sigma_own[t] < -0x1p-100f && s > -INFINITY && u < INFINITY;
-                }
-            } else if constexpr (STATS) {
-                nf_paper_net_body<Net, NT, 1, true>(acc, sigma_own, pe, dirf, Wi, Ci, act4, lane,
-                                                    NfMarkedPre<NfLivePre, COLS>{{st, wd, pf, ring_v, head_v, tail_v}, stats});
-            } else {
-                nf_paper_net_body<Net, NT, 1, true>(acc, sigma_own, pe, dirf, Wi, Ci, act4, lane, NfLivePre{st, wd, pf, ring_v, head_v, tail_v});
-            }
-            nf_live_mark<STATS, COLS>(stats, NF_LIVE_PH_TILE, NF_LIVE_PH_APPEND);
-            int lane_o = lane;
-            asm volatile("" : "+v"(lane_o));
-            const int g = lane_o >> 4, c = lane_o & 15;
-            unsigned live = 0;
-            int S_o = S;
-            asm volatile("" : "+v"(S_o));
-            const int64_t p0_o = (int64_t)(uint32_t)__builtin_amdgcn_readfirstlane((int)(uint32_t)p0_v) |
-                                 ((int64_t)__builtin_amdgcn_readfirstlane((int)(p0_v >> 32)) << 32);
-#pragma unroll
-            for (int t = 0; t < NT; ++t) {
-                const int64_t p = p0_o + 16 * t + c;
-                bool is_live;
-                if constexpr (GATE) {
-                    const bool last = (p + 1) % S_o == 0;
-                    is_live = g == 0 && p < n_points && (!proven[t] || last);
-                    tag_own[t] = __int_as_float(last ? 1 : 0);
-                } else {
-                    is_live = g == 0 && p < n_points && (!(sigma_own[t] <= 0.0f) || (p + 1) % S_o == 0);
-                }
-                live |= ((unsigned)__builtin_amdgcn_ballot_w64(is_live) & 0xffffu) << (16 * t);
-            }
-            const int head = __builtin_amdgcn_readfirstlane(head_v), cnt = head - __builtin_amdgcn_readfirstlane(tail_v);
-            const int n_live = __builtin_popcount(live);
-            live_v = (int)live;
-            if constexpr (GATE) {
-                const int64_t left = n_points - p0_o;
-                nf_live_stat<STATS, COLS>(stats, NF_GATE_STAT_PROVEN, (left < 16 * NT ? (int)left : 16 * NT) - n_live);
-            }
-            if (cnt + n_live >= 16 * NT) {
-                run_v = 1;
-            } else {
-                const __amdgpu_buffer_rsrc_t ring = nf_live_ring(ring_v);
-                unsigned mm = live;
-#pragma unroll 1
-                for (int i = 0; i < n_live; i += 4) {
-                    f32x4 v[4];
-                    int off[4];
-#pragma unroll
-                    for (int u = 0; u < 4; ++u) {
-                        const bool ok = i + u < n_live;
-                        const int r = ok ? nf_live_pop(mm) : 0;
-                        off[u] = ok ? ((head + i + u) & (NF_LIVE_ROWS - 1)) * 1024 + lane_o * 16 : NF_LIVE_OOB;
-                        v[u] = act4[nf_live_slab(r, lane_o)];
-                    }
-#pragma unroll
-                    for (int u = 0; u < 4; ++u) nf_live_store(ring, off[u], v[u]);
-                }
-#pragma unroll
-                for (int t = 0; t < NT; ++t) {
-                    const int bit = 16 * t + c;
-                    if ((live >> bit) & 1u) {
-                        const int row = (head + __builtin_popcount(live & ((1u << bit) - 1u))) & (NF_LIVE_ROWS - 1);
-                        nf_live_store(ring, NF_LIVE_DIR_B + row * 64 + g * 16, dirf[t][0]);
-                        if (g == 0) {
-                            const int64_t p = p0_o + bit;
-                            nf_live_store(ring, NF_LIVE_META_B + row * 16,
-                                          (f32x4){__int_as_float((int)(uint32_t)p), __int_as_float((int)(p >> 32)), GATE ? tag_own[t] : sigma_own[t], 0.0f});
-                        }
-                    }
-                }
-                head_v = head + n_live;
-                asm volatile("" : "+v"(head_v));
-            }
-            nf_live_mark<STATS, COLS>(stats, NF_LIVE_PH_APPEND, -1);
-        } else {
-            if constexpr (GATE) {
-                NfGatePre pre{st, pf, ring_v, head_v, tail_v, bound_v};
-                pre.wait();
-                pre.loads(Wi, Ci, lane);
-            } else {
-                NfLivePre pre{st, wd, pf, ring_v, head_v, tail_v};
-                pre.wait();
-                pre.loads(Wi, Ci, lane);
-            }
-#pragma unroll
-            for (int t = 0; t < NT; ++t) {
-                dirf[t][0] = (f32x4){0.0f, 0.0f, 0.0f, 0.0f};
-                sigma_own[t] = 0.0f;
-            }
-            run_v = __builtin_amdgcn_readfirstlane(head_v) != __builtin_amdgcn_readfirstlane(tail_v) ? 2 : 0;
-        }
-        asm volatile("" : "+v"(live_v), "+v"(run_v));
-        const int run = __builtin_amdgcn_readfirstlane(run_v);
-        if (run != 0) {
-            nf_live_stat<STATS, COLS>(stats, NF_LIVE_STAT_RUNS, 1);
-            if (run == 2) nf_live_stat<STATS, COLS>(stats, NF_LIVE_STAT_FLUSH, __builtin_amdgcn_readfirstlane(head_v) - __builtin_amdgcn_readfirstlane(tail_v));
-            nf_live_mark<STATS, COLS>(stats, -1, NF_LIVE_PH_ENTRY);
-            int lane_o = lane;
-            asm volatile("" : "+v"(lane_o));
-            const int g = lane_o >> 4, c = lane_o & 15;
-            const __amdgpu_buffer_rsrc_t ring = nf_live_ring(ring_v);
-            const int tail = __builtin_amdgcn_readfirstlane(tail_v), cnt = __builtin_amdgcn_readfirstlane(head_v) - tail;
-            const unsigned own = run == 1 ? (unsigned)__builtin_amdgcn_readfirstlane(live_v) : 0u;
-            const unsigned fill = run == 1 ? ~own : (1u << cnt) - 1u;
-            const int n_fill = __builtin_popcount(fill);
-            f32x4 meta[NT];
-            bool valid[NT];
-#pragma unroll
-            for (int t = 0; t < NT; ++t) {
-                const int bit = 16 * t + c;
-                const bool f = (fill >> bit) & 1u;
-                const int row = (tail + __builtin_popcount(fill & ((1u << bit) - 1u))) & (NF_LIVE_ROWS - 1);
-                const f32x4 fd = nf_live_load(ring, f ? NF_LIVE_DIR_B + row * 64 + g * 16 : NF_LIVE_OOB);
-                const f32x4 fm = nf_live_load(ring, f ? NF_LIVE_META_B + row * 16 : NF_LIVE_OOB);
-                const int64_t p = (p0_v) + bit;
-                dirf[t][0] = f ? fd : dirf[t][0];
-                meta[t] = f ? fm : (f32x4){__int_as_float((int)(uint32_t)p), __int_as_float((int)(p >> 32)), GATE ? tag_own[t] : sigma_own[t], 0.0f};
-                valid[t] = f || ((own >> bit) & 1u);
-            }
-            unsigned hh = fill;
-#pragma unroll
-            for (int i = 0; i < NF_LIVE_PF; ++i) {
-                if (i < n_fill) {
-                    const int h = nf_live_pop(hh);
-                    act4[nf_live_slab(h, lane_o)] = pf[i];
-                }
-            }
-#pragma unroll 1
-            for (int i = NF_LIVE_PF; i < n_fill; i += 4) {
-                f32x4 v[4];
-                int h[4];
-#pragma unroll
-                for (int u = 0; u < 4; ++u) {
-                    const bool ok = i + u < n_fill;
-                    h[u] = ok ? nf_live_pop(hh) : -1;
-                    v[u] = nf_live_load(ring, ok ? ((tail + i + u) & (NF_LIVE_ROWS - 1)) * 1024 + lane_o * 16 : NF_LIVE_OOB);
-                }
-#pragma unroll
-                for (int u = 0; u < 4; ++u)
-                    if (h[u] >= 0) act4[nf_live_slab(h[u], lane_o)] = v[u];
-            }
-            constexpr int NDIR = 1;
-            constexpr unsigned D0 = Net::OFF_D0 / 4;
-            nf_read_b<NT>(st.b0, act4, lane, 0);
-            nf_live_mark<STATS, COLS>(stats, NF_LIVE_PH_ENTRY, NF_LIVE_PH_RUN);
-            f32x4 acc[NT][16], bj[NT];
-            float sigma_raw[NT];
-            if constexpr (GATE) {
-                nf_seg_lds<NT, 16, true, true>(acc, st, Wi, Net::OFF_FEAT / 4, 16, act4, lane);
-                nf_pending_b<NT, true>(bj, st);
-                nf_tail<NT, 16, 16, 9, 1>(acc, st.wb, bj, st, Wi, D0, Ci, Net::B_D0, act4, lane);
-                NF_NET_COLOUR();
-            } else {
-                NF_NET_COLOUR_D0(8, 9, wd);
-                NF_NET_COLOUR_REST();
-            }
-            int lane_s = lane;
-            asm volatile("" : "+v"(lane_s));
-            if ((lane_s >> 4) == 0) {
-#pragma unroll
-                for (int t = 0; t < NT; ++t) {
-                    if (valid[t]) {
-                        const int64_t p = (int64_t)(uint32_t)__float_as_int(meta[t].x) | ((int64_t)__float_as_int(meta[t].y) << 32);
-                        if constexpr (GATE) {
-                            const bool keep = !(sigma_raw[t] <= 0.0f) || __float_as_int(meta[t].z) != 0;
-                            if (p >= 0 && p < n_points)
-                                raw_v[p] = (f32x4){keep ? acc[t][0].x : 0.0f, keep ? acc[t][0].y : 0.0f, keep ? acc[t][0].z : 0.0f, sigma_raw[t]};
-                        } else {
-                            if (p >= 0 && p < n_points) raw_v[p] = (f32x4){acc[t][0].x, acc[t][0].y, acc[t][0].z, meta[t].z};
-                        }
-                    }
-                }
-            }
-            tail_v = tail + n_fill;
-            asm volatile("" : "+v"(tail_v));
-            nf_live_mark<STATS, COLS>(stats, NF_LIVE_PH_RUN, -1);
-        }
-        asm volatile("" : "+v"(more_v));
-        if (__builtin_amdgcn_readfirstlane(more_v) == 0) break;
-        {
-            nf_live_mark<STATS, COLS>(stats, -1, NF_LIVE_PH_DEAD);
-            int lane_s = lane;
-            asm volatile("" : "+v"(lane_s));
-            const int g = lane_s >> 4, c = lane_s & 15;
-            asm volatile("" : "+v"(live_v));
-#pragma unroll
-            for (int t = 0; t < NT; ++t) {
-                const int64_t p = p0_v + 16 * t + c;
-                if (g == 0 && p < n_points && !(((unsigned)live_v >> (16 * t + c)) & 1u)) raw_v[p] = (f32x4){0.0f, 0.0f, 0.0f, sigma_own[t]};
-            }
-            nf_live_mark<STATS, COLS>(stats, NF_LIVE_PH_DEAD, -1);
-        }
-        asm volatile("" : "+v"(next_v));
-        unit_v = next_v;
-    }
-    nf_live_stat<STATS, COLS>(stats, NF_LIVE_STAT_CLOCK, (long long)wall_clock64(), true);
-}
+    for (int t = 0; t < NT; ++t) {
+        uint32_t p = p0 + 16 * t + c;
+        if (p >= np) p = np - 1u;
+        bool last;
+        uint32_t ray32;
+        const size_t q = nf_skip_map(p, np, n_full, S, last, ray32), ray = ray32;
+        qv[t] = (uint32_t)q | (last ? NF_SKIP_LAST_BIT : 0u);
+        const float zz = z[q];
+        const float dx = rd[ray * 3 + 0], dy = rd[ray * 3 + 1], dz = rd[ray * 3 + 2];
+        const float px = nf_add(ro[ray * 3 + 0], nf_mul(dx, zz));
+        const float py = nf_add(ro[ray * 3 + 1], nf_mul(dy, zz));
+        const float pz = nf_add(ro[ray * 3 + 2], nf_mul(dz, zz));
+        nf_encode_point(px, py, pz, g, pe[t]);
+        float s, cs;
+        nf_sincos(nf_mul(rd_view[ray * 3 + 2], (float)(1 << g)), &s, &cs);
+        dirf[t][0] = (f32x4){s, cs, 0.0f, 0.0f};
+    }
+}
+
+#define NF_LIVE_KERNEL k_paper_mlp_fwd_live
+#define NF_LIVE_SKIPLAST false
+#include "nf_mlp_live_kernel_text.inc"
+#undef NF_LIVE_KERNEL
+#undef NF_LIVE_SKIPLAST
+#define NF_LIVE_KERNEL k_paper_mlp_fwd_live_skip
+#define NF_LIVE_SKIPLAST true
+#include "nf_mlp_live_kernel_text.inc"
+#undef NF_LIVE_KERNEL
+#undef NF_LIVE_SKIPLAST
 
 static inline int64_t nf_live_grid_cap(int max_workgroups) {
     const int64_t cu = nf_cu_count();
@@ -448,14 +231,21 @@
     return reinterpret_cast<unsigned*>(p.base + (size_t)i * NF_LIVE_SLOT_B);
 }
 
-template <bool STATS, bool GATE = false>
+#define NF_SKIP_FACTORS 8
+int nf_skip_last_prepare(const float* ro, const float* rd, const float* z, int64_t n_rays, int n_samples, float* raw, const double* factors,
+                         unsigned* flag, hipStream_t stream);
+
+template <bool STATS, bool GATE = false, bool SKIPLAST = false>
 static inline int nf_live_launch(const float* packed, const float* cond, const float* ro, const float* rd, const float* rd_view, const float* z,
                                  int64_t n_rays, int n_samples, float* raw, float* scratch, size_t scratch_floats, int max_workgroups,
-                                 long long* stats, nf_stream_t stream, const float* bound = nullptr, bool clocks = false) {
+                                 long long* stats, nf_stream_t stream, const float* bound = nullptr, bool clocks = false,
+                                 const double* factors = nullptr) {
     static_assert(NF_MLP_WAVES * 16 * NF_MLP_NT == 128, "nf_mlp_fwd_launch sizes the grid for 128 points per workgroup");
     if (max_workgroups < 0 || !scratch || ((uintptr_t)scratch & 15) ||
         scratch_floats < (size_t)nf_live_grid_cap(max_workgroups) * NF_MLP_WAVES * (NF_LIVE_WAVE_B / 4) ||
         (GATE && (!bound || ((uintptr_t)bound & 15))))
+        return NF_EINVAL;
+    if (SKIPLAST && (!factors || ((uintptr_t)factors & 7) || (n_rays > 0 && (n_samples < 2 || n_rays > (((int64_t)1 << 31) - 64) / n_samples))))
         return NF_EINVAL;
     const float* rdv = rd_view ? rd_view : rd;
     if (STATS && clocks) stats = reinterpret_cast<long long*>((uintptr_t)stats | 1);
@@ -470,12 +260,19 @@
             rc = (int)hipErrorOutOfMemory;
             return;
         }
-        const hipError_t e = hipMemsetAsync(counter, 0, sizeof(unsigned), nf_s(stream));
+        const hipError_t e = hipMemsetAsync(counter, 0, (SKIPLAST ? 2 : 1) * sizeof(unsigned), nf_s(stream));
         if (e != hipSuccess) {
             rc = (int)e;
             return;
         }
         const int64_t cap = nf_live_grid_cap(max_workgroups);
+        if constexpr (SKIPLAST) {
+            rc = nf_skip_last_prepare(ro, rd, z, n_rays, n_samples, raw, factors, counter + 1, nf_s(stream));
+            if (rc) return;
+            hipLaunchKernelGGL((k_paper_mlp_fwd_live_skip<NF_MLP_NT, STATS, GATE>), dim3((unsigned)(grid < cap ? grid : cap)),
+                               dim3(64 * NF_MLP_WAVES), 0, nf_s(stream), packed, cond, ro, rd, rdv, z, n_points, n_samples, raw, scratch, counter,
+                               stats, bound);
+        } else
         hipLaunchKernelGGL((k_paper_mlp_fwd_live<NF_MLP_NT, STATS, GATE>), dim3((unsigned)(grid < cap ? grid : cap)), dim3(64 * NF_MLP_WAVES), 0,
                            nf_s(stream), packed, cond, ro, rd, rdv, z, n_points, n_samples, raw, scratch, counter, stats, bound);
     });
diff --git a/4d-facial-avatars_amd/csrc/nf_mlp_live_kernel_text.inc b/4d-facial-avatars_amd/csrc/nf_mlp_live_kernel_text.inc
--- /dev/null
+++ b/4d-facial-avatars_amd/csrc/nf_mlp_live_kernel_text.inc
@@ -0,0 +1,296 @@
+template <int NT, bool STATS, bool GATE = false>
+__global__ void __launch_bounds__(64 * NF_MLP_WAVES, 1)
+NF_LIVE_KERNEL(const float* __restrict__ packed, const float* __restrict__ cond_, const float* __restrict__ ro,
+               const float* __restrict__ rd, const float* __restrict__ rd_view, const float* __restrict__ z,
+               int64_t n_points, int S, float* __restrict__ raw, float* __restrict__ scratch, unsigned* __restrict__ counter,
+               long long* __restrict__ stats, const float* __restrict__ bound) {
+    constexpr bool SKIPLAST = NF_LIVE_SKIPLAST;
+    constexpr bool MARKS = STATS && !SKIPLAST;
+    using Net = NfPaperNet;
+    constexpr int COLS = GATE ? NF_GATE_STAT_COLS : NF_LIVE_STAT_COLS;
+    __shared__ __attribute__((aligned(16))) f32x4 lds[NF_MLP_WAVES * 16 * NT * 64];
+    const int lane = threadIdx.x & 63, wave = threadIdx.x >> 6;
+    f32x4* act4 = lds + wave * (16 * NT * 64);
+    typedef __attribute__((address_space(1))) f32x4 nf_gf32x4;
+    nf_gf32x4* raw_v = (nf_gf32x4*)raw;
+    asm volatile("" : "+v"(raw_v));
+    char* ring_v = reinterpret_cast<char*>(scratch) + ((size_t)blockIdx.x * NF_MLP_WAVES + wave) * NF_LIVE_WAVE_B;
+    asm volatile("" : "+v"(ring_v));
+    const float* z_v = z;
+    const float* rdv_v = rd_view;
+    asm volatile("" : "+v"(z_v), "+v"(rdv_v));
+    const float* bound_v = bound;
+    if constexpr (GATE) asm volatile("" : "+v"(bound_v));
+    int head_v = 0, tail_v = 0;
+    asm volatile("" : "+v"(head_v), "+v"(tail_v));
+    typedef __attribute__((address_space(1))) unsigned nf_gu32;
+    nf_gu32* ctr_v = (nf_gu32*)counter;
+    asm volatile("" : "+v"(ctr_v));
+    unsigned np_v = 0, nfull_v = 0;
+    int S_v = 0;
+    if constexpr (SKIPLAST) {
+        nfull_v = (unsigned)n_points;
+        S_v = S;
+        np_v = ctr_v[1] != 0u ? nfull_v : nfull_v - nfull_v / (unsigned)S;
+        asm volatile("" : "+v"(np_v), "+v"(nfull_v), "+v"(S_v));
+    }
+#define NF_SKIP_NP() ({ asm volatile("" : "+v"(np_v)); (uint32_t)__builtin_amdgcn_readfirstlane((int)np_v); })
+#define NF_SKIP_NFULL() ({ asm volatile("" : "+v"(nfull_v)); (uint32_t)__builtin_amdgcn_readfirstlane((int)nfull_v); })
+#define NF_SKIP_S() ({ asm volatile("" : "+v"(S_v)); __builtin_amdgcn_readfirstlane(S_v); })
+    unsigned unit_v = 0;
+    if (lane == 0) unit_v = __hip_atomic_fetch_add(ctr_v, 1u, __ATOMIC_RELAXED, __HIP_MEMORY_SCOPE_AGENT);
+    asm volatile("" : "+v"(unit_v));
+#pragma unroll 1
+    for (;;) {
+        const int64_t p0 = (int64_t)(uint32_t)__builtin_amdgcn_readfirstlane((int)unit_v) * (16 * NT);
+        int64_t p0_v = p0;
+        asm volatile("" : "+v"(p0_v));
+        int more_v;
+        if constexpr (SKIPLAST) more_v = p0 < (int64_t)NF_SKIP_NP();
+        else more_v = p0 < n_points;
+        asm volatile("" : "+v"(more_v));
+        const bool more = __builtin_amdgcn_readfirstlane(more_v) != 0;
+        unsigned next_v = 0;
+        if (more && lane == 0) next_v = __hip_atomic_fetch_add(ctr_v, 1u, __ATOMIC_RELAXED, __HIP_MEMORY_SCOPE_AGENT);
+        if (more) nf_live_stat<STATS, COLS>(stats, NF_LIVE_STAT_UNITS, 1);
+        int opaque0 = 0;
+        asm volatile("" : "+s"(opaque0));
+        const NfW Wi = nf_w_image(packed + opaque0, Net::PACKED), Ci = nf_w_image(cond_ + opaque0, Net::COND_FLOATS);
+        NfStream<NT> st;
+        f32x4 wd[16], pf[NF_LIVE_PF > 0 ? NF_LIVE_PF : 1];
+        f32x4 dirf[NT][1];
+        float sigma_own[NT];
+        float tag_own[NT] = {};
+        uint32_t qv[NT] = {};
+        bool proven[NT] = {};
+        int live_v = 0, run_v = 0;
+        if (more) {
+            nf_live_mark<MARKS, COLS>(stats, -1, NF_LIVE_PH_TRUNK);
+            f32x4 pe[NT][4];
+            if constexpr (SKIPLAST)
+                nf_net_inputs_skip<NT>(pe, dirf, qv, (uint32_t)p0, NF_SKIP_NP(), NF_SKIP_NFULL(), NF_SKIP_S(), lane, ro, rd, rdv_v, z_v);
+            else
+                nf_net_inputs<NT>(pe, dirf, p0, n_points, S, lane, ro, rd, rdv_v, z_v);
+            f32x4 acc[NT][16];
+            if constexpr (GATE) {
+                if constexpr (MARKS)
+                    nf_paper_net_body<Net, NT, 1, true, NfMarkedPre<NfGatePre, COLS>, true>(
+                        acc, sigma_own, pe, dirf, Wi, Ci, act4, lane, NfMarkedPre<NfGatePre, COLS>{{st, pf, ring_v, head_v, tail_v, bound_v}, stats});
+                else
+                    nf_paper_net_body<Net, NT, 1, true, NfGatePre, true>(acc, sigma_own, pe, dirf, Wi, Ci, act4, lane,
+                                                                         NfGatePre{st, pf, ring_v, head_v, tail_v, bound_v});
+#pragma unroll
+                for (int t = 0; t < NT; ++t) {
+                    const float s = acc[t][8].x, u = acc[t][8].y;
+                    sigma_own[t] = nf_add(s, nf_mul(u, 0x1p-13f));
+                    proven[t] = sigma_own[t] < -0x1p-100f && s > -INFINITY && u < INFINITY;
+                }
+            } else if constexpr (MARKS) {
+                nf_paper_net_body<Net, NT, 1, true>(acc, sigma_own, pe, dirf, Wi, Ci, act4, lane,
+                                                    NfMarkedPre<NfLivePre, COLS>{{st, wd, pf, ring_v, head_v, tail_v}, stats});
+            } else {
+                nf_paper_net_body<Net, NT, 1, true>(acc, sigma_own, pe, dirf, Wi, Ci, act4, lane, NfLivePre{st, wd, pf, ring_v, head_v, tail_v});
+            }
+            nf_live_mark<MARKS, COLS>(stats, NF_LIVE_PH_TILE, NF_LIVE_PH_APPEND);
+            int lane_o = lane;
+            asm volatile("" : "+v"(lane_o));
+            const int g = lane_o >> 4, c = lane_o & 15;
+            unsigned live = 0;
+            int S_o = S;
+            if constexpr (!SKIPLAST) asm volatile("" : "+v"(S_o));
+            const int64_t p0_o = (int64_t)(uint32_t)__builtin_amdgcn_readfirstlane((int)(uint32_t)p0_v) |
+                                 ((int64_t)__builtin_amdgcn_readfirstlane((int)(p0_v >> 32)) << 32);
+            const uint32_t np_o = SKIPLAST ? NF_SKIP_NP() : 0u;
+#pragma unroll
+            for (int t = 0; t < NT; ++t) {
+                const int64_t p = p0_o + 16 * t + c;
+                bool is_live;
+                if constexpr (SKIPLAST) {
+                    const bool last = (qv[t] & NF_SKIP_LAST_BIT) != 0u;
+                    const bool kept = GATE ? !proven[t] : !(sigma_own[t] <= 0.0f);
+                    is_live = g == 0 && (uint32_t)p < np_o && (kept || last);
+                    if constexpr (GATE) tag_own[t] = __int_as_float(last ? 1 : 0);
+                } else if constexpr (GATE) {
+                    const bool last = (p + 1) % S_o == 0;
+                    is_live = g == 0 && p < n_points && (!proven[t] || last);
+                    tag_own[t] = __int_as_float(last ? 1 : 0);
+                } else {
+                    is_live = g == 0 && p < n_points && (!(sigma_own[t] <= 0.0f) || (p + 1) % S_o == 0);
+                }
+                live |= ((unsigned)__builtin_amdgcn_ballot_w64(is_live) & 0xffffu) << (16 * t);
+            }
+            const int head = __builtin_amdgcn_readfirstlane(head_v), cnt = head - __builtin_amdgcn_readfirstlane(tail_v);
+            const int n_live = __builtin_popcount(live);
+            live_v = (int)live;
+            if constexpr (GATE) {
+                const int64_t left = (SKIPLAST ? (int64_t)np_o : n_points) - p0_o;
+                nf_live_stat<STATS, COLS>(stats, NF_GATE_STAT_PROVEN, (left < 16 * NT ? (int)left : 16 * NT) - n_live);
+            }
+            if (cnt + n_live >= 16 * NT) {
+                run_v = 1;
+            } else {
+                const __amdgpu_buffer_rsrc_t ring = nf_live_ring(ring_v);
+                unsigned mm = live;
+#pragma unroll 1
+                for (int i = 0; i < n_live; i += 4) {
+                    f32x4 v[4];
+                    int off[4];
+#pragma unroll
+                    for (int u = 0; u < 4; ++u) {
+                        const bool ok = i + u < n_live;
+                        const int r = ok ? nf_live_pop(mm) : 0;
+                        off[u] = ok ? ((head + i + u) & (NF_LIVE_ROWS - 1)) * 1024 + lane_o * 16 : NF_LIVE_OOB;
+                        v[u] = act4[nf_live_slab(r, lane_o)];
+                    }
+#pragma unroll
+                    for (int u = 0; u < 4; ++u) nf_live_store(ring, off[u], v[u]);
+                }
+#pragma unroll
+                for (int t = 0; t < NT; ++t) {
+                    const int bit = 16 * t + c;
+                    if ((live >> bit) & 1u) {
+                        const int row = (head + __builtin_popcount(live & ((1u << bit) - 1u))) & (NF_LIVE_ROWS - 1);
+                        nf_live_store(ring, NF_LIVE_DIR_B + row * 64 + g * 16, dirf[t][0]);
+                        if (g == 0) {
+                            int64_t p = p0_o + bit;
+                            if constexpr (SKIPLAST) p = qv[t] & ~NF_SKIP_LAST_BIT;
+                            nf_live_store(ring, NF_LIVE_META_B + row * 16,
+                                          (f32x4){__int_as_float((int)(uint32_t)p), __int_as_float((int)(p >> 32)), GATE ? tag_own[t] : sigma_own[t], 0.0f});
+                        }
+                    }
+                }
+                head_v = head + n_live;
+                asm volatile("" : "+v"(head_v));
+            }
+            nf_live_mark<MARKS, COLS>(stats, NF_LIVE_PH_APPEND, -1);
+        } else {
+            if constexpr (GATE) {
+                NfGatePre pre{st, pf, ring_v, head_v, tail_v, bound_v};
+                pre.wait();
+                pre.loads(Wi, Ci, lane);
+            } else {
+                NfLivePre pre{st, wd, pf, ring_v, head_v, tail_v};
+                pre.wait();
+                pre.loads(Wi, Ci, lane);
+            }
+#pragma unroll
+            for (int t = 0; t < NT; ++t) {
+                dirf[t][0] = (f32x4){0.0f, 0.0f, 0.0f, 0.0f};
+                sigma_own[t] = 0.0f;
+            }
+            run_v = __builtin_amdgcn_readfirstlane(head_v) != __builtin_amdgcn_readfirstlane(tail_v) ? 2 : 0;
+        }
+        asm volatile("" : "+v"(live_v), "+v"(run_v));
+        const int run = __builtin_amdgcn_readfirstlane(run_v);
+        if (run != 0) {
+            nf_live_stat<STATS, COLS>(stats, NF_LIVE_STAT_RUNS, 1);
+            if (run == 2) nf_live_stat<STATS, COLS>(stats, NF_LIVE_STAT_FLUSH, __builtin_amdgcn_readfirstlane(head_v) - __builtin_amdgcn_readfirstlane(tail_v));
+            nf_live_mark<MARKS, COLS>(stats, -1, NF_LIVE_PH_ENTRY);
+            int lane_o = lane;
+            asm volatile("" : "+v"(lane_o));
+            const int g = lane_o >> 4, c = lane_o & 15;
+            const __amdgpu_buffer_rsrc_t ring = nf_live_ring(ring_v);
+            const int tail = __builtin_amdgcn_readfirstlane(tail_v), cnt = __builtin_amdgcn_readfirstlane(head_v) - tail;
+            const unsigned own = run == 1 ? (unsigned)__builtin_amdgcn_readfirstlane(live_v) : 0u;
+            const unsigned fill = run == 1 ? ~own : (1u << cnt) - 1u;
+            const int n_fill = __builtin_popcount(fill);
+            f32x4 meta[NT];
+            bool valid[NT];
+#pragma unroll
+            for (int t = 0; t < NT; ++t) {
+                const int bit = 16 * t + c;
+                const bool f = (fill >> bit) & 1u;
+                const int row = (tail + __builtin_popcount(fill & ((1u << bit) - 1u))) & (NF_LIVE_ROWS - 1);
+                const f32x4 fd = nf_live_load(ring, f ? NF_LIVE_DIR_B + row * 64 + g * 16 : NF_LIVE_OOB);
+                const f32x4 fm = nf_live_load(ring, f ? NF_LIVE_META_B + row * 16 : NF_LIVE_OOB);
+                int64_t p = (p0_v) + bit;
+                if constexpr (SKIPLAST) p = qv[t] & ~NF_SKIP_LAST_BIT;
+                dirf[t][0] = f ? fd : dirf[t][0];
+                meta[t] = f ? fm : (f32x4){__int_as_float((int)(uint32_t)p), __int_as_float((int)(p >> 32)), GATE ? tag_own[t] : sigma_own[t], 0.0f};
+                valid[t] = f || ((own >> bit) & 1u);
+            }
+            unsigned hh = fill;
+#pragma unroll
+            for (int i = 0; i < NF_LIVE_PF; ++i) {
+                if (i < n_fill) {
+                    const int h = nf_live_pop(hh);
+                    act4[nf_live_slab(h, lane_o)] = pf[i];
+                }
+            }
+#pragma unroll 1
+            for (int i = NF_LIVE_PF; i < n_fill; i += 4) {
+                f32x4 v[4];
+                int h[4];
+#pragma unroll
+                for (int u = 0; u < 4; ++u) {
+                    const bool ok = i + u < n_fill;
+                    h[u] = ok ? nf_live_pop(hh) : -1;
+                    v[u] = nf_live_load(ring, ok ? ((tail + i + u) & (NF_LIVE_ROWS - 1)) * 1024 + lane_o * 16 : NF_LIVE_OOB);
+                }
+#pragma unroll
+                for (int u = 0; u < 4; ++u)
+                    if (h[u] >= 0) act4[nf_live_slab(h[u], lane_o)] = v[u];
+            }
+            constexpr int NDIR = 1;
+            constexpr unsigned D0 = Net::OFF_D0 / 4;
+            nf_read_b<NT>(st.b0, act4, lane, 0);
+            nf_live_mark<MARKS, COLS>(stats, NF_LIVE_PH_ENTRY, NF_LIVE_PH_RUN);
+            f32x4 acc[NT][16], bj[NT];
+            float sigma_raw[NT];
+            if constexpr (GATE) {
+                nf_seg_lds<NT, 16, true, true>(acc, st, Wi, Net::OFF_FEAT / 4, 16, act4, lane);
+                nf_pending_b<NT, true>(bj, st);
+                nf_tail<NT, 16, 16, 9, 1>(acc, st.wb, bj, st, Wi, D0, Ci, Net::B_D0, act4, lane);
+                NF_NET_COLOUR();
+            } else {
+                NF_NET_COLOUR_D0(8, 9, wd);
+                NF_NET_COLOUR_REST();
+            }
+            int lane_s = lane;
+            asm volatile("" : "+v"(lane_s));
+            if ((lane_s >> 4) == 0) {
+#pragma unroll
+                for (int t = 0; t < NT; ++t) {
+                    if (valid[t]) {
+                        const int64_t p = (int64_t)(uint32_t)__float_as_int(meta[t].x) | ((int64_t)__float_as_int(meta[t].y) << 32);
+                        if constexpr (GATE) {
+                            const bool keep = !(sigma_raw[t] <= 0.0f) || __float_as_int(meta[t].z) != 0;
+                            if (p >= 0 && p < (SKIPLAST ? (int64_t)NF_SKIP_NFULL() : n_points))
+                                raw_v[p] = (f32x4){keep ? acc[t][0].x : 0.0f, keep ? acc[t][0].y : 0.0f, keep ? acc[t][0].z : 0.0f, sigma_raw[t]};
+                        } else {
+                            if (p >= 0 && p < (SKIPLAST ? (int64_t)NF_SKIP_NFULL() : n_points)) raw_v[p] = (f32x4){acc[t][0].x, acc[t][0].y, acc[t][0].z, meta[t].z};
+                        }
+                    }
+                }
+            }
+            tail_v = tail + n_fill;
+            asm volatile("" : "+v"(tail_v));
+            nf_live_mark<MARKS, COLS>(stats, NF_LIVE_PH_RUN, -1);
+        }
+        asm volatile("" : "+v"(more_v));
+        if (__builtin_amdgcn_readfirstlane(more_v) == 0) break;
+        {
+            nf_live_mark<MARKS, COLS>(stats, -1, NF_LIVE_PH_DEAD);
+            int lane_s = lane;
+            asm volatile("" : "+v"(lane_s));
+            const int g = lane_s >> 4, c = lane_s & 15;
+            asm volatile("" : "+v"(live_v));
+#pragma unroll
+            for (int t = 0; t < NT; ++t) {
+                const int64_t p = p0_v + 16 * t + c;
+                if constexpr (SKIPLAST) {
+                    const uint32_t np = NF_SKIP_NP(), q = qv[t] & ~NF_SKIP_LAST_BIT;
+                    if (g == 0 && (uint32_t)p < np && !(((unsigned)live_v >> (16 * t + c)) & 1u)) raw_v[q] = (f32x4){0.0f, 0.0f, 0.0f, sigma_own[t]};
+                } else
+                if (g == 0 && p < n_points && !(((unsigned)live_v >> (16 * t + c)) & 1u)) raw_v[p] = (f32x4){0.0f, 0.0f, 0.0f, sigma_own[t]};
+            }
+            nf_live_mark<MARKS, COLS>(stats, NF_LIVE_PH_DEAD, -1);
+        }
+        asm volatile("" : "+v"(next_v));
+        unit_v = next_v;
+    }
+    nf_live_stat<STATS, COLS>(stats, NF_LIVE_STAT_CLOCK, (long long)wall_clock64(), true);
+#undef NF_SKIP_NP
+#undef NF_SKIP_NFULL
+#undef NF_SKIP_S
+}
diff --git a/4d-facial-avatars_amd/csrc/nf_mlp_live_skip.hip b/4d-facial-avatars_amd/csrc/nf_mlp_live_skip.hip
--- /dev/null
+++ b/4d-facial-avatars_amd/csrc/nf_mlp_live_skip.hip
@@ -0,0 +1,8 @@
+#include "nf_mlp_live_kernel.h"
+
+extern "C" int nf_paper_mlp_fwd_live_skip(const float* packed, const double* factors, const float* cond, const float* ro, const float* rd,
+                                          const float* rd_view, const float* z, int64_t n_rays, int n_samples, float* raw, float* scratch,
+                                          size_t scratch_floats, int max_workgroups, nf_stream_t stream) {
+    return nf_live_launch<false, false, true>(packed, cond, ro, rd, rd_view, z, n_rays, n_samples, raw, scratch, scratch_floats, max_workgroups,
+                                              nullptr, stream, nullptr, false, factors);
+}
diff --git a/4d-facial-avatars_amd/csrc/nf_mlp_live_skip_stats.hip b/4d-facial-avatars_amd/csrc/nf_mlp_live_skip_stats.hip
--- /dev/null
+++ b/4d-facial-avatars_amd/csrc/nf_mlp_live_skip_stats.hip
@@ -0,0 +1,13 @@
+#include "nf_mlp_live_kernel.h"
+
+extern "C" int nf_paper_mlp_fwd_live_skip_stats(const float* packed, const double* factors, const float* cond, const float* ro, const float* rd,
+                                                const float* rd_view, const float* z, int64_t n_rays, int n_samples, float* raw,
+                                                float* scratch, size_t scratch_floats, int max_workgroups, int64_t* stats, size_t stats_rows,
+                                                nf_stream_t stream) {
+    static_assert(sizeof(long long) == sizeof(int64_t), "a statistics row is int64s");
+    if (max_workgroups < 0 || !stats || ((uintptr_t)stats & 7) || stats_rows < (size_t)nf_live_grid_cap(max_workgroups) * NF_MLP_WAVES) return NF_EINVAL;
+    const hipError_t e = hipMemsetAsync(stats, 0, stats_rows * NF_LIVE_STAT_COLS * sizeof(int64_t), nf_s(stream));
+    if (e != hipSuccess) return (int)e;
+    return nf_live_launch<true, false, true>(packed, cond, ro, rd, rd_view, z, n_rays, n_samples, raw, scratch, scratch_floats, max_workgroups,
+                                             reinterpret_cast<long long*>(stats), stream, nullptr, false, factors);
+}
diff --git a/4d-facial-avatars_amd/csrc/nf_mlp_skip_last.hip b/4d-facial-avatars_amd/csrc/nf_mlp_skip_last.hip
--- /dev/null
+++ b/4d-facial-avatars_amd/csrc/nf_mlp_skip_last.hip
@@ -0,0 +1,98 @@
+#include "nf_mlp_live_kernel.h"
+
+__host__ __device__ static inline float nf_skip_rmax(const double* f) {
+    double G = 1.0;
+    for (int l = 0; l < NF_SKIP_FACTORS; ++l) G *= f[l];
+    if (!(G <= 0x1p120)) return 0.0f;
+    const double q = 0x1p120 / G;
+    float r = (float)q;
+    if ((double)r > q) r = nextafterf(r, 0.0f);
+    return r;
+}
+
+__device__ __forceinline__ double nf_skip_nanmax(double a, double b) { return (b > a || b != b) ? b : a; }
+
+__global__ void __launch_bounds__(1024) k_paper_skip_last_factors(const float* __restrict__ packed, const float* __restrict__ cond,
+                                                                  double* __restrict__ factors) {
+    using Net = NfPaperNet;
+    __shared__ double sa[4][256], sc[256];
+    const int l = blockIdx.x, n = threadIdx.x & 255, part = threadIdx.x >> 8;
+    double a = 0.0;
+    if (l < 7) {
+        const int off = l == 0 ? Net::OFF_L0 : l == 1 ? Net::OFF_L1 : l == 2 ? Net::OFF_L2 : l == 3 ? Net::OFF_L3 : l == 4 ? Net::OFF_L4
+                        : l == 5 ? Net::OFF_L5 : Net::OFF_FEAT;
+        const int nk = l == 0 ? 4 : (l == 3 ? 20 : 16), no = n >> 4, i = n & 15;
+        for (int ni = part; ni < nk; ni += 4)
+            for (int g = 0; g < 4; ++g) {
+                const float4 w = *reinterpret_cast<const float4*>(packed + off + (((ni * 16 + no) * 64) + g * 16 + i) * 4);
+                a += fabs((double)w.x) + fabs((double)w.y) + fabs((double)w.z) + fabs((double)w.w);
+            }
+        if (part == 0) sc[n] = fabs((double)cond[256 * l + n]);
+    } else if (part == 0) {
+        a = fabs((double)packed[Net::OFF_D0 + (((n >> 4) * 9 + 8) * 64 + ((n >> 2) & 3) * 16) * 4 + (n & 3)]);
+        for (int j = n; j < Net::COND_FLOATS; j += 256)
+            if (!(fabsf(cond[j]) < INFINITY)) a = NAN;
+        sc[n] = n == 0 ? fabs((double)cond[Net::B_D0 + 128]) : 0.0;
+    }
+    sa[part][n] = a;
+    __syncthreads();
+    if (part == 0) sa[0][n] = ((sa[0][n] + sa[1][n]) + sa[2][n]) + sa[3][n];
+    __syncthreads();
+    for (int h = 128; h > 0; h >>= 1) {
+        if (part == 0 && n < h) {
+            sa[0][n] = l < 7 ? nf_skip_nanmax(sa[0][n], sa[0][n + h]) : sa[0][n] + sa[0][n + h];
+            sc[n] = nf_skip_nanmax(sc[n], sc[n + h]);
+        }
+        __syncthreads();
+    }
+    if (threadIdx.x == 0) {
+        const double f = sa[0][0] + sc[0];
+        factors[l] = f >= 1.0 ? f : (f != f ? f : 1.0);
+    }
+}
+
+__global__ void __launch_bounds__(256) k_paper_skip_last_pre(const float* __restrict__ ro, const float* __restrict__ rd, const float* __restrict__ z,
+                                                             int64_t n_rays, int S, float4* __restrict__ raw, const double* __restrict__ factors,
+                                                             unsigned* __restrict__ flag) {
+    __shared__ float rmax_s;
+    if (threadIdx.x == 0) rmax_s = nf_skip_rmax(factors);
+    __syncthreads();
+    const int64_t ray = (int64_t)blockIdx.x * 256 + threadIdx.x;
+    if (ray >= n_rays) return;
+    const float rmax = rmax_s;
+    const int64_t last = ray * S + (S - 1);
+    const float dx = rd[ray * 3 + 0], dy = rd[ray * 3 + 1], dz = rd[ray * 3 + 2], zz = z[last];
+    const float n2 = nf_add(nf_add(nf_mul(dx, dx), nf_mul(dy, dy)), nf_mul(dz, dz));
+    const float px = nf_add(ro[ray * 3 + 0], nf_mul(dx, zz));
+    const float py = nf_add(ro[ray * 3 + 1], nf_mul(dy, zz));
+    const float pz = nf_add(ro[ray * 3 + 2], nf_mul(dz, zz));
+    const bool ok = rmax > 0.0f && n2 >= 0x1p-12f && fabsf(px) <= rmax && fabsf(py) <= rmax && fabsf(pz) <= rmax;
+    raw[last] = make_float4(0.0f, 0.0f, 0.0f, 0.0f);
+    if (!ok) *flag = 1u;
+}
+
+int nf_skip_last_prepare(const float* ro, const float* rd, const float* z, int64_t n_rays, int n_samples, float* raw, const double* factors,
+                         unsigned* flag, hipStream_t stream) {
+    const int64_t grid = (n_rays + 255) / 256;
+    if (grid <= 0 || grid > 0x7fffffff) return NF_EINVAL;
+    hipLaunchKernelGGL(k_paper_skip_last_pre, dim3((unsigned)grid), dim3(256), 0, stream, ro, rd, z, n_rays, n_samples,
+                       reinterpret_cast<float4*>(raw), factors, flag);
+    NF_RETURN_LAUNCH();
+}
+
+extern "C" size_t nf_paper_skip_last_factors(void) { return NF_SKIP_FACTORS; }
+
+extern "C" int nf_paper_skip_last_bound(const float* packed, const float* cond, double* factors, nf_stream_t stream) {
+    if (!packed || !cond || !factors || ((uintptr_t)factors & 7) || ((uintptr_t)packed & 15)) return NF_EINVAL;
+    hipLaunchKernelGGL(k_paper_skip_last_factors, dim3(NF_SKIP_FACTORS), dim3(1024), 0, nf_s(stream), packed, cond, factors);
+    NF_RETURN_LAUNCH();
+}
+
+extern "C" float nf_paper_skip_last_rmax(const double* factors_host) { return factors_host ? nf_skip_rmax(factors_host) : 0.0f; }
+
+extern "C" int nf_paper_mlp_fwd_gated_skip(const float* packed, const float* bound, const double* factors, const float* cond, const float* ro,
+                                           const float* rd, const float* rd_view, const float* z, int64_t n_rays, int n_samples, float* raw,
+                                           float* scratch, size_t scratch_floats, int max_workgroups, nf_stream_t stream) {
+    return nf_live_launch<false, true, true>(packed, cond, ro, rd, rd_view, z, n_rays, n_samples, raw, scratch, scratch_floats, max_workgroups,
+                                             nullptr, stream, bound, false, factors);
+}
diff --git a/4d-facial-avatars_amd/csrc/nf_mlp_skip_last_stats.hip b/4d-facial-avatars_amd/csrc/nf_mlp_skip_last_stats.hip
--- /dev/null
+++ b/4d-facial-avatars_amd/csrc/nf_mlp_skip_last_stats.hip
@@ -0,0 +1,13 @@
+#include "nf_mlp_live_kernel.h"
+
+extern "C" int nf_paper_mlp_fwd_gated_skip_stats(const float* packed, const float* bound, const double* factors, const float* cond,
+                                                 const float* ro, const float* rd, const float* rd_view, const float* z, int64_t n_rays,
+                                                 int n_samples, float* raw, float* scratch, size_t scratch_floats, int max_workgroups,
+                                                 int64_t* stats, size_t stats_rows, nf_stream_t stream) {
+    static_assert(sizeof(long long) == sizeof(int64_t), "a statistics row is int64s");
+    if (max_workgroups < 0 || !stats || ((uintptr_t)stats & 7) || stats_rows < (size_t)nf_live_grid_cap(max_workgroups) * NF_MLP_WAVES) return NF_EINVAL;
+    const hipError_t e = hipMemsetAsync(stats, 0, stats_rows * NF_GATE_STAT_COLS * sizeof(int64_t), nf_s(stream));
+    if (e != hipSuccess) return (int)e;
+    return nf_live_launch<true, true, true>(packed, cond, ro, rd, rd_view, z, n_rays, n_samples, raw, scratch, scratch_floats, max_workgroups,
+                                            reinterpret_cast<long long*>(stats), stream, bound, false, factors);
+}
diff --git a/4d-facial-avatars_amd/nerf/_hip.py b/4d-facial-avatars_amd/nerf/_hip.py
--- a/4d-facial-avatars_amd/nerf/_hip.py
+++ b/4d-facial-avatars_amd/nerf/_hip.py
@@ -192,6 +192,13 @@
 _PROTOTYPES["nf_paper_mlp_fwd_live_phases"] = _PROTOTYPES["nf_paper_mlp_fwd_live_stats"]
 _PROTOTYPES["nf_paper_mlp_fwd_gated_stats"] = (C.c_int, [_P, _P, _P, _P, _P, _P, _P, _L, _I, _P, _P, _Z, _I, _P, _Z, _P])
 _PROTOTYPES["nf_paper_mlp_fwd_gated_phases"] = _PROTOTYPES["nf_paper_mlp_fwd_gated_stats"]
+_PROTOTYPES["nf_paper_skip_last_factors"] = (_Z, [])
+_PROTOTYPES["nf_paper_skip_last_bound"] = (C.c_int, [_P, _P, _P, _P])
+_PROTOTYPES["nf_paper_skip_last_rmax"] = (C.c_float, [_P])
+_PROTOTYPES["nf_paper_mlp_fwd_gated_skip"] = (C.c_int, [_P, _P, _P, _P, _P, _P, _P, _P, _L, _I, _P, _P, _Z, _I, _P])
+_PROTOTYPES["nf_paper_mlp_fwd_gated_skip_stats"] = (C.c_int, [_P, _P, _P, _P, _P, _P, _P, _P, _L, _I, _P, _P, _Z, _I, _P, _Z, _P])
+_PROTOTYPES["nf_paper_mlp_fwd_live_skip"] = (C.c_int, [_P, _P, _P, _P, _P, _P, _P, _L, _I, _P, _P, _Z, _I, _P])
+_PROTOTYPES["nf_paper_mlp_fwd_live_skip_stats"] = (C.c_int, [_P, _P, _P, _P, _P, _P, _P, _L, _I, _P, _P, _Z, _I, _P, _Z, _P])
 _PROTOTYPES["nf_isosurface_workspace_bytes"] = (_Z, [_I, _I, _I])
 _PROTOTYPES["nf_isosurface_count"] = (C.c_int, [_P, _I, _I, _I, _F, _P, _Z, _P, _P])
 _PROTOTYPES["nf_isosurface_emit"] = (C.c_int, [_P, _I, _I, _I, _F, _P, _P, _P, _Z, _P, _L, _P, _L, _P, _P])
diff --git a/4d-facial-avatars_amd/nerf/models.py b/4d-facial-avatars_amd/nerf/models.py
--- a/4d-facial-avatars_amd/nerf/models.py
+++ b/4d-facial-avatars_amd/nerf/models.py
@@ -22,17 +22,21 @@
             hw = self._hip_weights = ops.MLPWeights(self.FAMILY, params)
         return hw
 
-    def hip_forward(self, ro, rd, z, rd_view, expr, latent, near, far, need_grad, live_only=False):
+    def hip_forward(self, ro, rd, z, rd_view, expr, latent, near, far, need_grad, live_only=False, skip_last=False):
         ops.check_conditioning(expr, latent)
         fam, hw, prec = self.FAMILY, self.hip_weights(), ops.get_mlp_precision()
         fam.require_precision(prec)
+        if skip_last and not live_only:
+            raise ValueError("skip_last is an option of the live_only kernels")
         if live_only:
             if need_grad or not ops.live_colour_kernel(fam):
                 raise ValueError("live_only is an exact-f32 inference option of the families in ops.LIVE_FAMILIES (ops.live_colour_kernel)")
             packed = hw.get()
             if live_only == "gated":
-                return ops.mlp_fwd_gated(fam, packed, hw.get_bound(), ops.mlp_condition(fam, packed, expr, latent, near, far), ro, rd, z, rd_view), None
-            return ops.mlp_fwd_live(fam, packed, ops.mlp_condition(fam, packed, expr, latent, near, far), ro, rd, z, rd_view), None
+                return ops.mlp_fwd_gated(fam, packed, hw.get_bound(), ops.mlp_condition(fam, packed, expr, latent, near, far), ro, rd, z, rd_view,
+                                         skip_last=skip_last), None
+            return ops.mlp_fwd_live(fam, packed, ops.mlp_condition(fam, packed, expr, latent, near, far), ro, rd, z, rd_view,
+                                    skip_last=skip_last), None
         packed = hw.get()
         cond = ops.mlp_condition(fam, packed, expr, latent, near, far)
         if need_grad:
diff --git a/4d-facial-avatars_amd/nerf/ops.py b/4d-facial-avatars_amd/nerf/ops.py
--- a/4d-facial-avatars_amd/nerf/ops.py
+++ b/4d-facial-avatars_amd/nerf/ops.py
@@ -369,7 +369,7 @@
     return _live_launches[0]
 
 
-def mlp_fwd_live(fam: MLPFamily, packed, cond, ro, rd, z, rd_view=None, max_workgroups: int = 0) -> torch.Tensor:
+def mlp_fwd_live(fam: MLPFamily, packed, cond, ro, rd, z, rd_view=None, max_workgroups: int = 0, skip_last: bool = False) -> torch.Tensor:
     if fam.prefix not in LIVE_FAMILIES:
         raise NotImplementedError(f"the {fam.prefix} model family has no live-colour kernel")
     dev = H.require_device(packed, cond, ro, rd, z, rd_view)
@@ -380,8 +380,14 @@
         scratch = _LIVE_SCRATCH.get(key)
         if scratch is None:
             scratch = _LIVE_SCRATCH[key] = torch.empty(fam.fn("mlp_fwd_live_scratch_floats")(int(max_workgroups)), dtype=torch.float32, device=dev)
-        fam.call("mlp_fwd_live", H.ptr(packed), H.ptr(cond), H.ptr(ro), H.ptr(rd), H.ptr(rd_view), H.ptr(z), n_rays, n_samples, H.ptr(raw),
-                 H.ptr(scratch), scratch.numel(), int(max_workgroups), H.stream_ptr(dev))
+        if skip_last and n_samples >= 2:
+            fam.call("mlp_fwd_live_skip", H.ptr(packed), H.ptr(skip_last_factors(fam, packed, cond)), H.ptr(cond), H.ptr(ro), H.ptr(rd),
+                     H.ptr(rd_view), H.ptr(z), n_rays, n_samples, H.ptr(raw), H.ptr(scratch), scratch.numel(), int(max_workgroups),
+                     H.stream_ptr(dev))
+            _skip_last_launches[0] += 1
+        else:
+            fam.call("mlp_fwd_live", H.ptr(packed), H.ptr(cond), H.ptr(ro), H.ptr(rd), H.ptr(rd_view), H.ptr(z), n_rays, n_samples, H.ptr(raw),
+                     H.ptr(scratch), scratch.numel(), int(max_workgroups), H.stream_ptr(dev))
     _live_launches[0] += 1
     return raw
 
@@ -447,7 +453,7 @@
              H.ptr(scratch), scratch.numel(), int(max_workgroups), *tail)
 
 
-def mlp_fwd_gated(fam: MLPFamily, packed, bound, cond, ro, rd, z, rd_view=None, max_workgroups: int = 0) -> torch.Tensor:
+def mlp_fwd_gated(fam: MLPFamily, packed, bound, cond, ro, rd, z, rd_view=None, max_workgroups: int = 0, skip_last: bool = False) -> torch.Tensor:
     if fam.prefix not in LIVE_FAMILIES:
         raise NotImplementedError(f"the {fam.prefix} model family has no gated kernel")
     dev = H.require_device(packed, bound, cond, ro, rd, z, rd_view)
@@ -458,7 +464,13 @@
         scratch = _LIVE_SCRATCH.get(key)
         if scratch is None:
             scratch = _LIVE_SCRATCH[key] = torch.empty(fam.fn("mlp_fwd_live_scratch_floats")(int(max_workgroups)), dtype=torch.float32, device=dev)
-        _gated_call("mlp_fwd_gated", fam, packed, bound, cond, ro, rd, z, rd_view, max_workgroups, scratch, raw, H.stream_ptr(dev))
+        if skip_last and n_samples >= 2:
+            fam.call("mlp_fwd_gated_skip", H.ptr(packed), H.ptr(bound), H.ptr(skip_last_factors(fam, packed, cond)), H.ptr(cond), H.ptr(ro),
+                     H.ptr(rd), H.ptr(rd_view), H.ptr(z), n_rays, n_samples, H.ptr(raw), H.ptr(scratch), scratch.numel(), int(max_workgroups),
+                     H.stream_ptr(dev))
+            _skip_last_launches[0] += 1
+        else:
+            _gated_call("mlp_fwd_gated", fam, packed, bound, cond, ro, rd, z, rd_view, max_workgroups, scratch, raw, H.stream_ptr(dev))
     _gated_launches[0] += 1
     return raw
 
@@ -476,6 +488,40 @@
         _gated_call("mlp_fwd_gated_phases", fam, packed, bound, cond, ro, rd, z, rd_view, max_workgroups, scratch, raw, stats.data_ptr(), waves,
                     H.stream_ptr(dev))
     return raw, stats
+
+
+SKIP_LAST_PASSES_DEFAULT = ("coarse", "fine")
+_skip_last_passes = (set(SKIP_LAST_PASSES_DEFAULT) if os.environ.get("NERFACE_SKIP_LAST") is None
+                     else {p for p in os.environ["NERFACE_SKIP_LAST"].split(",") if p in ("coarse", "fine")})
+_skip_last_launches = [0]
+
+
+def set_skip_last(on, passes=("coarse", "fine")) -> None:
+    global _skip_last_passes
+    _skip_last_passes = set(SKIP_LAST_PASSES_DEFAULT) if on is None else (set(passes) if on else set())
+
+
+def skip_last_applies(which: str, live, bg, n_samples: int) -> bool:
+    return bool(live) and bg is not None and n_samples >= 2 and which in _skip_last_passes
+
+
+def skip_last_launches() -> int:
+    return _skip_last_launches[0]
+
+
+def skip_last_factors(fam: MLPFamily, packed, cond) -> torch.Tensor:
+    if fam.prefix not in LIVE_FAMILIES:
+        raise NotImplementedError(f"the {fam.prefix} model family has no live-colour kernel")
+    dev = H.require_device(packed, cond)
+    factors = torch.empty(fam.fn("skip_last_factors")(), dtype=torch.float64, device=dev)
+    with torch.cuda.device(dev):
+        fam.call("skip_last_bound", H.ptr(packed), H.ptr(cond), H.ptr(factors), H.stream_ptr(dev))
+    return factors
+
+
+def skip_last_rmax(fam: MLPFamily, factors) -> float:
+    host = factors.detach().cpu().contiguous()
+    return float(fam.fn("skip_last_rmax")(host.data_ptr()))
 
 
 _SIGMA_ENTRY = {"f32": "mlp_sigma", "bf16x3": "mlp_sigma_bf16", "f16x3": "mlp_sigma_f16", "f16x2": "mlp_sigma_f16x2"}
diff --git a/4d-facial-avatars_amd/nerf/train_utils.py b/4d-facial-avatars_amd/nerf/train_utils.py
--- a/4d-facial-avatars_amd/nerf/train_utils.py
+++ b/4d-facial-avatars_amd/nerf/train_utils.py
@@ -56,13 +56,15 @@
             raw_c = state_c = rgb_c = None
             disp_c, acc_c, w_c = ops.volume_weights_fwd(model_c.hip_sigma(ro, rd, z_c, expr, lat_d, near, far), z_c, rd, noise_c)
         else:
-            raw_c, state_c = model_c.hip_forward(ro, rd, z_c, rd_view, expr, lat_d, near, far, need_grad, live_only=live_c)
+            raw_c, state_c = model_c.hip_forward(ro, rd, z_c, rd_view, expr, lat_d, near, far, need_grad, live_only=live_c,
+                                                 skip_last=ops.skip_last_applies("coarse", live_c, bg, nc))
             rgb_c, disp_c, acc_c, w_c = ops.volume_render_fwd(raw_c, z_c, rd, noise_c, bg, white)
         outs = [rgb_c, disp_c, acc_c]
         ctx.has_fine = nf > 0 and model_f is not None
         if ctx.has_fine:
             z_f = ops.resample_merge(z_c, w_c, nf, u)
-            raw_f, state_f = model_f.hip_forward(ro, rd, z_f, rd_view, expr, lat_d, near, far, need_grad, live_only=live_f)
+            raw_f, state_f = model_f.hip_forward(ro, rd, z_f, rd_view, expr, lat_d, near, far, need_grad, live_only=live_f,
+                                                 skip_last=ops.skip_last_applies("fine", live_f, bg, z_f.shape[1]))
             rgb_f, disp_f, acc_f, w_f = ops.volume_render_fwd(raw_f, z_f, rd, noise_f, bg, white)
             w_last = w_f[:, -1].contiguous()
             outs += [rgb_f, disp_f, acc_f, w_last]
diff --git a/include/nerface_hip.h b/include/nerface_hip.h
--- a/include/nerface_hip.h
+++ b/include/nerface_hip.h
@@ -413,6 +413,23 @@
                                  const float* rd_view, const float* z, int64_t n_rays, int n_samples, float* raw, float* scratch,
                                  size_t scratch_floats, int max_workgroups, int64_t* stats, size_t stats_rows, nf_stream_t stream);
 
+size_t nf_paper_skip_last_factors(void);
+int nf_paper_skip_last_bound(const float* packed, const float* cond, double* factors, nf_stream_t stream);
+float nf_paper_skip_last_rmax(const double* factors_host);
+int nf_paper_mlp_fwd_gated_skip(const float* packed, const float* bound, const double* factors, const float* cond, const float* ro,
+                                const float* rd, const float* rd_view, const float* z, int64_t n_rays, int n_samples, float* raw,
+                                float* scratch, size_t scratch_floats, int max_workgroups, nf_stream_t stream);
+int nf_paper_mlp_fwd_gated_skip_stats(const float* packed, const float* bound, const double* factors, const float* cond, const float* ro,
+                                      const float* rd, const float* rd_view, const float* z, int64_t n_rays, int n_samples, float* raw,
+                                      float* scratch, size_t scratch_floats, int max_workgroups, int64_t* stats, size_t stats_rows,
+                                      nf_stream_t stream);
+int nf_paper_mlp_fwd_live_skip(const float* packed, const double* factors, const float* cond, const float* ro, const float* rd,
+                               const float* rd_view, const float* z, int64_t n_rays, int n_samples, float* raw, float* scratch,
+                               size_t scratch_floats, int max_workgroups, nf_stream_t stream);
+int nf_paper_mlp_fwd_live_skip_stats(const float* packed, const double* factors, const float* cond, const float* ro, const float* rd,
+                                     const float* rd_view, const float* z, int64_t n_rays, int n_samples, float* raw, float* scratch,
+                                     size_t scratch_floats, int max_workgroups, int64_t* stats, size_t stats_rows, nf_stream_t stream);
+
 size_t nf_isosurface_workspace_bytes(int nx, int ny, int nz);
 int nf_isosurface_count(const float* grid, int nx, int ny, int nz, float level, void* workspace, size_t workspace_bytes,
                         int64_t* counts_dev, nf_stream_t stream);
```

After: 627,700 rays/s, median of 6. About the same (+0.8%).
